# enp1s0/tsqr-gpu

Hardware: AMD Instinct MI355X
Metric: tsqr_gflops (higher is better)
Workload: dtype f32; 1 GPU; c2: M=2^20 x N=64 per GPU, fp32_tc_cor, reorth=0, U(-1,1); global 1048576 x 64 (weak scaling); F_QR=4MN^2-4/3N^3; R-factor engine: gram_bf16x3_cholesky; engine=gram_bf16x3_cholesky, m_per_gpu=1048576, n=64, mode=fp32_tc_cor, reorthogonalize=False, parallelism=row-partitioned x1

## Files before the change

### include/tsqr_mi.h

```cpp
#ifndef TSQR_MI_H
#define TSQR_MI_H
#include <stddef.h>

#ifdef __cplusplus
extern "C" {
#endif

enum tsqr_mi_compute_mode {
	TSQR_MI_FP16_NOTC = 0,
	TSQR_MI_FP16_TC_NOCOR = 1,
	TSQR_MI_FP32_NOTC = 2,
	TSQR_MI_FP32_TC_COR = 3,
	TSQR_MI_FP32_TC_NOCOR = 4,
	TSQR_MI_MIXED_TC_COR_EMU = 5,
	TSQR_MI_TF32_TC_COR = 6,
	TSQR_MI_TF32_TC_COR_EMU = 7,
	TSQR_MI_TF32_TC_NOCOR = 8,
	TSQR_MI_TF32_TC_NOCOR_EMU = 9
};

#define TSQR_MI_SUCCESS               0
#define TSQR_MI_ERROR_INVALID_SIZE    1
#define TSQR_MI_ERROR_UNSUPPORTED     2
#define TSQR_MI_ERROR_NOT_FINITE      3

int tsqr_mi_version(void);
const char* tsqr_mi_last_error(void);

size_t tsqr_mi_working_q_size(size_t m, size_t n);
size_t tsqr_mi_working_r_size(size_t m, size_t n);
size_t tsqr_mi_working_l_size(size_t m);
size_t tsqr_mi_working_reorth_size(size_t m);
size_t tsqr_mi_batch_size_log2(size_t m);
size_t tsqr_mi_batch_size(size_t m);

int tsqr_mi_qr_f32(int mode, int reorth,
                   float* q, size_t ldq, float* r, size_t ldr, float* a, size_t lda,
                   size_t m, size_t n,
                   void* wq, void* wr, float* reorth_w, unsigned* d_wl, unsigned* h_wl,
                   void* stream);
typedef struct tsqr_mi_ticket {
	int state;
	int pending;
	int slot;
	int own_flag;
	unsigned seq;
	unsigned verdict;
	float scond;
	int mode, reorth;
	float *q, *r, *a;
	size_t ldq, ldr, lda, m, n;
	void *wq, *wr, *stream;
	unsigned *h_wl, *words, *words_dev;
} tsqr_mi_ticket;
int tsqr_mi_qr_f32_submit(int mode, int reorth,
                          float* q, size_t ldq, float* r, size_t ldr, float* a, size_t lda,
                          size_t m, size_t n,
                          void* wq, void* wr, float* reorth_w, unsigned* d_wl, unsigned* h_wl,
                          void* stream, tsqr_mi_ticket* ticket);
int tsqr_mi_qr_f32_finish(tsqr_mi_ticket* ticket);

int tsqr_mi_qr_f32_loop(int count, int mode, int reorth,
                        float* q, size_t ldq, float* r, size_t ldr, float* a, size_t lda,
                        size_t m, size_t n,
                        void* wq, void* wr, float* reorth_w, unsigned* d_wl, unsigned* h_wl,
                        void* stream);
void tsqr_mi_set_loop_depth(int depth);

int tsqr_mi_qr_f32_batch(int count, int mode, int reorth,
                         float* const* q, size_t ldq, float* const* r, size_t ldr, float* const* a, size_t lda,
                         size_t m, size_t n,
                         void* wq, void* wr, float* reorth_w, unsigned* d_wl, unsigned* h_wl,
                         void* stream, int* states);

size_t tsqr_mi_working_q_size_f16(size_t m, size_t n);
size_t tsqr_mi_working_r_size_f16(size_t m, size_t n);
int tsqr_mi_qr_f16(int mode, int reorth,
                   void* q, size_t ldq, void* r, size_t ldr, const void* a, size_t lda,
                   size_t m, size_t n,
                   void* wq, void* wr, void* reorth_w, unsigned* d_wl, unsigned* h_wl,
                   void* stream);
int tsqr_mi_qr_f16_loop(int count, int mode, int reorth,
                        void* q, size_t ldq, void* r, size_t ldr, const void* a, size_t lda,
                        size_t m, size_t n,
                        void* wq, void* wr, void* reorth_w, unsigned* d_wl, unsigned* h_wl,
                        void* stream);

int tsqr_mi_qr_f16_batch(int count, int mode, int reorth,
                         void* const* q, size_t ldq, void* const* r, size_t ldr, const void* const* a, size_t lda,
                         size_t m, size_t n,
                         void* wq, void* wr, void* reorth_w, unsigned* d_wl, unsigned* h_wl,
                         void* stream, int* states);

int tsqr_mi_local_r_f32(float* r, size_t ldr, const float* a, size_t lda, size_t m, size_t n,
                        void* wq, void* wr, void* stream);
int tsqr_mi_apply_rinv_f32(int mode, float* q, size_t ldq, const float* a, size_t lda,
                           const float* r, size_t ldr, size_t m, size_t n,
                           void* wq, void* stream);
size_t tsqr_mi_gram_elems(size_t n);
int tsqr_mi_gram_f32(int level, double* gsum, const float* a, size_t lda, size_t m, size_t n, void* wq, void* wr, void* stream);
int tsqr_mi_chol_f32(int level, float* r, size_t ldr, const double* gsum, size_t m, size_t n, void* wq, unsigned* status_out, void* stream);
int tsqr_mi_chol_status(const void* wq, size_t m, size_t n, unsigned* status_out, void* stream);
int tsqr_mi_stream_wait(void* stream);
int tsqr_mi_apply_z_f32(int mode, float* q, size_t ldq, const float* a, size_t lda, size_t m, size_t n, void* wq, void* stream);
int tsqr_mi_rmul_f32(float* r, size_t ldr, const float* r2, size_t ldr2, size_t n, void* wq, void* stream);

size_t tsqr_mi_working_q_size_dist(size_t m_local, size_t n, int nranks);
size_t tsqr_mi_working_r_size_dist(size_t m_local, size_t n, int nranks);
int tsqr_mi_qr_f32_dist(int mode, int reorth,
                        float* q, size_t ldq, float* r, size_t ldr, float* a, size_t lda,
                        size_t m_local, size_t n,
                        void* wq, void* wr, float* gather_buf ,
                        void* nccl_comm, int nranks, void* stream);
int tsqr_mi_qr_f32_dist_fn(int mode, int reorth,
                           float* q, size_t ldq, float* r, size_t ldr, float* a, size_t lda,
                           size_t m_local, size_t n,
                           void* wq, void* wr, float* gather_buf ,
                           void* nccl_comm, void* nccl_allreduce_fn, void* nccl_allgather_fn, int nranks, void* stream);
int tsqr_mi_qr_f32_dist_fn_loop(int count, int mode, int reorth,
                                float* q, size_t ldq, float* r, size_t ldr, float* a, size_t lda,
                                size_t m_local, size_t n,
                                void* wq, void* wr, float* gather_buf,
                                void* nccl_comm, void* nccl_allreduce_fn, void* nccl_allgather_fn, int nranks, void* stream);
int tsqr_mi_qr_f32_dist_fn_batch(int count, int mode, int reorth,
                                 float* const* q, size_t ldq, float* const* r, size_t ldr, float* const* a, size_t lda,
                                 size_t m_local, size_t n,
                                 void* wq, void* wr, float* gather_buf,
                                 void* nccl_comm, void* nccl_allreduce_fn, void* nccl_allgather_fn, int nranks, void* stream, int* states);
typedef int (*tsqr_mi_allreduce_f64_cb)(void* user, double* buf , size_t count, void* stream);
typedef int (*tsqr_mi_allgather_f32_cb)(void* user, const float* send , float* recv , size_t count, void* stream);
int tsqr_mi_qr_f32_dist_cb(int mode, int reorth,
                           float* q, size_t ldq, float* r, size_t ldr, float* a, size_t lda,
                           size_t m_local, size_t n,
                           void* wq, void* wr, float* gather_buf,
                           tsqr_mi_allreduce_f64_cb allreduce, tsqr_mi_allgather_f32_cb allgather, void* user, int nranks, void* stream);
int tsqr_mi_qr_f32_dist_cb_loop(int count, int mode, int reorth,
                                float* q, size_t ldq, float* r, size_t ldr, float* a, size_t lda,
                                size_t m_local, size_t n,
                                void* wq, void* wr, float* gather_buf,
                                tsqr_mi_allreduce_f64_cb allreduce, tsqr_mi_allgather_f32_cb allgather, void* user, int nranks, void* stream);
int tsqr_mi_qr_f32_dist_cb_batch(int count, int mode, int reorth,
                                 float* const* q, size_t ldq, float* const* r, size_t ldr, float* const* a, size_t lda,
                                 size_t m_local, size_t n,
                                 void* wq, void* wr, float* gather_buf,
                                 tsqr_mi_allreduce_f64_cb allreduce, tsqr_mi_allgather_f32_cb allgather, void* user, int nranks, void* stream, int* states);

size_t tsqr_mi_working_q_size_f64(size_t m, size_t n);
size_t tsqr_mi_working_r_size_f64(size_t m, size_t n);
int tsqr_mi_qr_f64(int reorth, double* q, size_t ldq, double* r, size_t ldr, double* a, size_t lda,
                   size_t m, size_t n, void* wq, void* wr, void* stream);
int tsqr_mi_last_sweeps_f64(void);

size_t tsqr_mi_working_q_size_f64_wide(size_t m, size_t n);
size_t tsqr_mi_working_r_size_f64_wide(size_t m, size_t n);
int tsqr_mi_qr_f64_wide(int reorth, double* q, size_t ldq, double* r, size_t ldr, double* a, size_t lda,
                        size_t m, size_t n, void* wq, void* wr, void* stream);

int tsqr_mi_validate_f32(const float* q, size_t ldq, const float* r, size_t ldr, const float* a, size_t lda,
                         size_t m, size_t n, double* scratch, double* out_host, double* gram_out_host, void* stream);

void tsqr_mi_profile_enable(int on);
int tsqr_mi_profile_read(double* ms, long* launches, int max_classes);

void tsqr_mi_set_policy(int policy);
int tsqr_mi_last_engine(void);

void tsqr_mi_set_tuning(int level0_waves, int tree_chunks_per_wave);
void tsqr_mi_set_tuning2(int gram_waves, int apply_waves);

#ifdef __cplusplus
}
#endif
#endif
```

### tsqr_gpu_amd/blockqr.py

```python
import ctypes
import enum
import os

_HERE = os.path.dirname(os.path.abspath(__file__))
LIB_PATH = os.environ.get("TSQR_MI_LIB") or os.path.join(_HERE, "csrc", "libtsqr_mi.so")


class compute_mode(enum.IntEnum):
    fp16_notc = 0
    fp16_tc_nocor = 1
    fp32_notc = 2
    fp32_tc_cor = 3
    fp32_tc_nocor = 4
    mixed_tc_cor_emu = 5
    tf32_tc_cor = 6
    tf32_tc_cor_emu = 7
    tf32_tc_nocor = 8
    tf32_tc_nocor_emu = 9


tsqr_colmun_size = 16
success_factorization = 0
error_invalid_matrix_size = 1
error_unsupported_mode = 2
error_not_finite = 3

C_ABI_SYMBOLS = [
    "tsqr_mi_version", "tsqr_mi_last_error",
    "tsqr_mi_working_q_size", "tsqr_mi_working_r_size", "tsqr_mi_working_l_size",
    "tsqr_mi_working_reorth_size", "tsqr_mi_batch_size_log2", "tsqr_mi_batch_size",
    "tsqr_mi_qr_f32", "tsqr_mi_local_r_f32", "tsqr_mi_apply_rinv_f32", "tsqr_mi_rmul_f32",
    "tsqr_mi_qr_f32_dist", "tsqr_mi_set_tuning", "tsqr_mi_profile_enable", "tsqr_mi_profile_read",
    "tsqr_mi_set_policy", "tsqr_mi_last_engine", "tsqr_mi_set_tuning2",
    "tsqr_mi_gram_elems", "tsqr_mi_gram_f32", "tsqr_mi_chol_f32", "tsqr_mi_chol_status", "tsqr_mi_stream_wait", "tsqr_mi_apply_z_f32", "tsqr_mi_validate_f32",
    "tsqr_mi_working_q_size_dist", "tsqr_mi_working_r_size_dist", "tsqr_mi_qr_f32_dist_cb",
    "tsqr_mi_qr_f32_loop", "tsqr_mi_qr_f32_dist_fn", "tsqr_mi_qr_f32_dist_fn_loop", "tsqr_mi_qr_f32_dist_cb_loop",
    "tsqr_mi_qr_f16", "tsqr_mi_qr_f16_loop", "tsqr_mi_working_q_size_f16", "tsqr_mi_working_r_size_f16",
    "tsqr_mi_qr_f32_submit", "tsqr_mi_qr_f32_finish", "tsqr_mi_set_loop_depth", "tsqr_mi_qr_f32_batch", "tsqr_mi_qr_f16_batch",
    "tsqr_mi_qr_f32_dist_fn_batch", "tsqr_mi_qr_f32_dist_cb_batch",
    "tsqr_mi_qr_f64", "tsqr_mi_working_q_size_f64", "tsqr_mi_working_r_size_f64", "tsqr_mi_last_sweeps_f64",
    "tsqr_mi_qr_f64_wide", "tsqr_mi_working_q_size_f64_wide", "tsqr_mi_working_r_size_f64_wide",
]


class Ticket(ctypes.Structure):
    _fields_ = [("state", ctypes.c_int), ("pending", ctypes.c_int), ("slot", ctypes.c_int), ("own_flag", ctypes.c_int), ("seq", ctypes.c_uint),
                ("verdict", ctypes.c_uint), ("scond", ctypes.c_float), ("mode", ctypes.c_int), ("reorth", ctypes.c_int),
                ("q", ctypes.c_void_p), ("r", ctypes.c_void_p), ("a", ctypes.c_void_p),
                ("ldq", ctypes.c_size_t), ("ldr", ctypes.c_size_t), ("lda", ctypes.c_size_t), ("m", ctypes.c_size_t), ("n", ctypes.c_size_t),
                ("wq", ctypes.c_void_p), ("wr", ctypes.c_void_p), ("stream", ctypes.c_void_p),
                ("h_wl", ctypes.c_void_p), ("words", ctypes.c_void_p), ("words_dev", ctypes.c_void_p)]

    def __del__(self):
        if self.pending == 0:
            return
        import sys
        import threading
        if _lib is not None and not sys.is_finalizing() and getattr(self, "_tid", None) == threading.get_ident():
            _lib.tsqr_mi_qr_f32_finish(ctypes.byref(self))
        else:
            import warnings
            warnings.warn("tsqr_gpu_amd: a Ticket in flight was dropped on another thread (or at shutdown) without finish(); "
                          "call blockqr.finish(ticket) on the submitting thread", ResourceWarning, stacklevel=2)


FP16_MODES = (compute_mode.fp16_notc, compute_mode.fp16_tc_nocor)

_lib = None


def lib():
    global _lib
    if _lib is not None:
        return _lib
    if not os.path.exists(LIB_PATH):
        raise RuntimeError(
            "tsqr_gpu_amd: %s is missing -- build it with `python -c 'import __graft_entry__ as g; g.build()'` "
            "or `make -C tsqr_gpu_amd/csrc`. There is no CPU fallback." % LIB_PATH)
    import torch
    L = ctypes.CDLL(LIB_PATH)
    sz, vp, ci = ctypes.c_size_t, ctypes.c_void_p, ctypes.c_int
    L.tsqr_mi_version.restype = ci
    L.tsqr_mi_last_error.restype = ctypes.c_char_p
    for name, args in [("tsqr_mi_working_q_size", [sz, sz]), ("tsqr_mi_working_r_size", [sz, sz]),
                       ("tsqr_mi_working_l_size", [sz]), ("tsqr_mi_working_reorth_size", [sz]),
                       ("tsqr_mi_batch_size_log2", [sz]), ("tsqr_mi_batch_size", [sz])]:
        getattr(L, name).restype = sz
        getattr(L, name).argtypes = args
    L.tsqr_mi_qr_f32.restype = ci
    L.tsqr_mi_qr_f32.argtypes = [ci, ci, vp, sz, vp, sz, vp, sz, sz, sz, vp, vp, vp, vp, vp, vp]
    L.tsqr_mi_local_r_f32.restype = ci
    L.tsqr_mi_local_r_f32.argtypes = [vp, sz, vp, sz, sz, sz, vp, vp, vp]
    L.tsqr_mi_apply_rinv_f32.restype = ci
    L.tsqr_mi_apply_rinv_f32.argtypes = [ci, vp, sz, vp, sz, vp, sz, sz, sz, vp, vp]
    L.tsqr_mi_gram_elems.restype = sz
    L.tsqr_mi_gram_elems.argtypes = [sz]
    L.tsqr_mi_gram_f32.restype = ci
    L.tsqr_mi_gram_f32.argtypes = [ci, vp, vp, sz, sz, sz, vp, vp, vp]
    L.tsqr_mi_chol_f32.restype = ci
    L.tsqr_mi_chol_f32.argtypes = [ci, vp, sz, vp, sz, sz, vp, ctypes.POINTER(ctypes.c_uint), vp]
    L.tsqr_mi_chol_status.restype = ci
    L.tsqr_mi_chol_status.argtypes = [vp, sz, sz, ctypes.POINTER(ctypes.c_uint), vp]
    L.tsqr_mi_stream_wait.restype = ci
    L.tsqr_mi_stream_wait.argtypes = [vp]
    L.tsqr_mi_apply_z_f32.restype = ci
    L.tsqr_mi_apply_z_f32.argtypes = [ci, vp, sz, vp, sz, sz, sz, vp, vp]
    L.tsqr_mi_validate_f32.restype = ci
    L.tsqr_mi_validate_f32.argtypes = [vp, sz, vp, sz, vp, sz, sz, sz, vp, ctypes.POINTER(ctypes.c_double), ctypes.POINTER(ctypes.c_double), vp]
    L.tsqr_mi_rmul_f32.restype = ci
    L.tsqr_mi_rmul_f32.argtypes = [vp, sz, vp, sz, sz, vp, vp]
    L.tsqr_mi_qr_f32_dist.restype = ci
    L.tsqr_mi_qr_f32_dist.argtypes = [ci, ci, vp, sz, vp, sz, vp, sz, sz, sz, vp, vp, vp, vp, ci, vp]
    L.tsqr_mi_qr_f32_dist_cb.restype = ci
    L.tsqr_mi_qr_f32_dist_cb.argtypes = [ci, ci, vp, sz, vp, sz, vp, sz, sz, sz, vp, vp, vp, vp, vp, vp, ci, vp]
    L.tsqr_mi_qr_f32_loop.restype = ci
    L.tsqr_mi_qr_f32_loop.argtypes = [ci] + L.tsqr_mi_qr_f32.argtypes
    L.tsqr_mi_qr_f32_submit.restype = ci
    L.tsqr_mi_qr_f32_submit.argtypes = L.tsqr_mi_qr_f32.argtypes + [ctypes.POINTER(Ticket)]
    L.tsqr_mi_qr_f32_finish.restype = ci
    L.tsqr_mi_qr_f32_finish.argtypes = [ctypes.POINTER(Ticket)]
    L.tsqr_mi_qr_f32_batch.restype = ci
    L.tsqr_mi_qr_f32_batch.argtypes = [ci, ci, ci, vp, sz, vp, sz, vp, sz, sz, sz, vp, vp, vp, vp, vp, vp, vp]
    L.tsqr_mi_qr_f16_batch.restype = ci
    L.tsqr_mi_qr_f16_batch.argtypes = L.tsqr_mi_qr_f32_batch.argtypes
    L.tsqr_mi_set_loop_depth.restype = None
    L.tsqr_mi_set_loop_depth.argtypes = [ci]
    L.tsqr_mi_qr_f16.restype = ci
    L.tsqr_mi_qr_f16.argtypes = L.tsqr_mi_qr_f32.argtypes
    L.tsqr_mi_qr_f16_loop.restype = ci
    L.tsqr_mi_qr_f16_loop.argtypes = [ci] + L.tsqr_mi_qr_f32.argtypes
    for name in ("tsqr_mi_working_q_size_f16", "tsqr_mi_working_r_size_f16"):
        getattr(L, name).restype = sz
        getattr(L, name).argtypes = [sz, sz]
    L.tsqr_mi_qr_f32_dist_fn.restype = ci
    L.tsqr_mi_qr_f32_dist_fn.argtypes = [ci, ci, vp, sz, vp, sz, vp, sz, sz, sz, vp, vp, vp, vp, vp, vp, ci, vp]
    L.tsqr_mi_qr_f32_dist_fn_loop.restype = ci
    L.tsqr_mi_qr_f32_dist_fn_loop.argtypes = [ci] + L.tsqr_mi_qr_f32_dist_fn.argtypes
    L.tsqr_mi_qr_f32_dist_cb_loop.restype = ci
    L.tsqr_mi_qr_f32_dist_cb_loop.argtypes = [ci] + L.tsqr_mi_qr_f32_dist_cb.argtypes
    L.tsqr_mi_qr_f32_dist_fn_batch.restype = ci
    L.tsqr_mi_qr_f32_dist_fn_batch.argtypes = [ci, ci, ci, vp, sz, vp, sz, vp, sz, sz, sz, vp, vp, vp, vp, vp, vp, ci, vp, vp]
    L.tsqr_mi_qr_f32_dist_cb_batch.restype = ci
    L.tsqr_mi_qr_f32_dist_cb_batch.argtypes = [ci, ci, ci, vp, sz, vp, sz, vp, sz, sz, sz, vp, vp, vp, vp, vp, vp, ci, vp, vp]
    for name in ("tsqr_mi_working_q_size_dist", "tsqr_mi_working_r_size_dist"):
        getattr(L, name).restype = sz
        getattr(L, name).argtypes = [sz, sz, ci]
    L.tsqr_mi_profile_enable.restype = None
    L.tsqr_mi_profile_enable.argtypes = [ci]
    L.tsqr_mi_profile_read.restype = ci
    L.tsqr_mi_profile_read.argtypes = [ctypes.POINTER(ctypes.c_double), ctypes.POINTER(ctypes.c_long), ci]
    L.tsqr_mi_set_policy.restype = None
    L.tsqr_mi_set_policy.argtypes = [ci]
    L.tsqr_mi_last_engine.restype = ci
    L.tsqr_mi_set_tuning2.restype = None
    L.tsqr_mi_set_tuning2.argtypes = [ci, ci]
    L.tsqr_mi_set_tuning.restype = None
    L.tsqr_mi_set_tuning.argtypes = [ci, ci]
    for name in ("tsqr_mi_working_q_size_f64", "tsqr_mi_working_r_size_f64", "tsqr_mi_working_q_size_f64_wide", "tsqr_mi_working_r_size_f64_wide"):
        getattr(L, name).restype = sz
        getattr(L, name).argtypes = [sz, sz]
    for name in ("tsqr_mi_qr_f64", "tsqr_mi_qr_f64_wide"):
        getattr(L, name).restype = ci
        getattr(L, name).argtypes = [ci, vp, sz, vp, sz, vp, sz, sz, sz, vp, vp, vp]
    L.tsqr_mi_last_sweeps_f64.restype = ci
    L.tsqr_mi_last_sweeps_f64.argtypes = []
    _lib = L
    return L


def last_error():
    return lib().tsqr_mi_last_error().decode()


def get_working_q_size(m, n):
    return lib().tsqr_mi_working_q_size(m, n)


def get_working_r_size(m, n):
    return lib().tsqr_mi_working_r_size(m, n)


def get_working_l_size(m):
    return lib().tsqr_mi_working_l_size(m)
# ... 336 lines not shown
```

### tsqr_gpu_amd/csrc/tsqr_kernels.hip

```cpp
#include <hip/hip_runtime.h>
#include <stdint.h>
#include <type_traits>
#include <utility>

namespace tsqrmi {

typedef float f32x4 __attribute__((ext_vector_type(4)));
typedef float f32x4u __attribute__((ext_vector_type(4), aligned(4)));
typedef short bf16x8 __attribute__((ext_vector_type(8)));
typedef _Float16 f16x8 __attribute__((ext_vector_type(8)));
typedef _Float16 f16x4 __attribute__((ext_vector_type(4)));

__device__ __forceinline__ void lds_barrier() { asm volatile("s_waitcnt lgkmcnt(0)\n\ts_barrier" ::: "memory"); }

template <int I, int N, class F>
__device__ __forceinline__ void static_for(F&& f) {
	if constexpr (I < N) {
		f(std::integral_constant<int, I>{});
		static_for<I + 1, N>(f);
	}
}

template <int K>
__device__ __forceinline__ float bcast16(float x) {
// ... 425 lines not shown

	float p[NT][16];
	const int ch_end = min(a.nchunks, (gw + 1) * a.cpw);
	int ch_first = gw * a.cpw;
	if (TRI && ch_first < ch_end) {
		load_chunk<NT>(p, a.src, a.ld, (size_t)ch_first * 64, a.m, a.n, c, q);
#pragma unroll
		for (int ct = 0; ct < NT; ct++)
#pragma unroll
			for (int rho = 0; rho < 16; rho++) {
				const int row = 16 * (rho >> 2) + 4 * q + (rho & 3), col = 16 * ct + c;
				if (col >= row) Rw[row * NP - (row * (row - 1)) / 2 + col - row] = p[ct][rho];
			}
		ch_first++;
		__builtin_amdgcn_wave_barrier();
	}
	for (int ch = ch_first; ch < ch_end; ch++) {
		load_chunk<NT>(p, a.src, a.ld, (size_t)ch * 64, a.m, a.n, c, q);
		fold_one<NT, TRI, COR>(p, Rw, Tl, a.n, c, q);
	}
	store_packed_r<NP>(a.dst + (size_t)gw * a.rows_store, a.dst_ld, Rw, a.rows_store, a.cols_store, lane);
}

struct FoldTreeArgs {
	const float* src; size_t ld;
	int nblocks, n;
	float* dst; size_t dst_ld;
	int rows_store, cols_store;
};
constexpr int FOLD_COOP_LDS_FLOATS = FOLD_COOP_WAVES * ((64 * 65) / 2 + 16) + FOLD_COOP_WAVES * 256 + 2 * FOLD_COOP_WAVES * 64 + 3 * FOLD_COOP_WAVES * 256;
template <bool COR>
__global__ __launch_bounds__(64 * FOLD_COOP_WAVES) void fold_coop_kernel(const FoldTreeArgs a) {
	constexpr int NT = 4, NP = 64, WAVES = FOLD_COOP_WAVES;
	constexpr int RP = (NP * (NP + 1)) / 2 + 16;
	extern __shared__ __attribute__((aligned(16))) char coop_smem[];
	float* Rs = reinterpret_cast<float*>(coop_smem);
	float* Ts = Rs + WAVES * RP;
	CoopCtx cc;
	cc.xd = Ts + WAVES * 256;
	cc.xw = cc.xd + 2 * WAVES * 64;
	const int lane = threadIdx.x & 63;
	const int wv = __builtin_amdgcn_readfirstlane(threadIdx.x >> 6);
	cc.wave = wv; cc.step = 0;
	const int c = lane & 15, q = lane >> 4;
	float* Rw = Rs + wv * RP;
	float* Tl = Ts + wv * 256;
	for (int i = lane; i < RP; i += 64) Rw[i] = 0.0f;
	const int first = blockIdx.x * WAVES;
	const size_t mrows = (size_t)a.nblocks * 64;
	float p[NT][16];
	load_chunk<NT, true>(p, a.src, a.ld, (size_t)first * 64, mrows, a.n, c, q);
#pragma unroll
	for (int ct = 0; ct < NT; ct++)
#pragma unroll
		for (int rho = 0; rho < 16; rho++) {
			const int row = 16 * (rho >> 2) + 4 * q + (rho & 3), col = 16 * ct + c;
			if (col >= row) Rw[row * NP - (row * (row - 1)) / 2 + col - row] = p[ct][rho];
		}
	if (wv > 0 && first + wv < a.nblocks) {
		load_chunk<NT, true>(p, a.src, a.ld, (size_t)(first + wv) * 64, mrows, a.n, c, q);
	} else {
#pragma unroll
		for (int ct = 0; ct < NT; ct++)
#pragma unroll
			for (int rho = 0; rho < 16; rho++) p[ct][rho] = 0.0f;
	}
	__builtin_amdgcn_wave_barrier();
	fold_one<NT, true, COR, true>(p, Rw, Tl, a.n, c, q, &cc);
	if (wv == 0) store_packed_r<NP>(a.dst + (size_t)blockIdx.x * a.rows_store, a.dst_ld, Rw, a.rows_store, a.cols_store, lane);
}

typedef double f64x4 __attribute__((ext_vector_type(4)));

__device__ __forceinline__ void part_store(double* p, double v) { __builtin_nontemporal_store(v, p); }
__device__ __forceinline__ double part_load(const double* p) { return __builtin_nontemporal_load(p); }

struct GramArgs {
	const float* a; size_t lda; size_t m; int n;
	int nchunks; int cpw; int nwaves;
	double* part;
	const unsigned* skip_status;
	unsigned* announce; unsigned announce_seq;
	int old_share;
};

__device__ __forceinline__ void announce_previous_call(unsigned* word, unsigned seq) {
	if (word && blockIdx.x == 0 && threadIdx.x == 0) *reinterpret_cast<volatile unsigned*>(word) = seq;
}

template <int NT>
__global__ __launch_bounds__(256) void gram_kernel(const GramArgs a) {
	constexpr int NTRI = (NT * (NT + 1)) / 2;
	__shared__ double red[2][NTRI * 256];
	announce_previous_call(a.announce, a.announce_seq);
	if (a.skip_status && a.skip_status[0] != 0) return;
	const int lane = threadIdx.x & 63;
	const int wv = threadIdx.x >> 6;
	const int gw = blockIdx.x * 4 + wv;
	const int c = lane & 15, q = lane >> 4;
	f64x4 acc[NTRI];
#pragma unroll
	for (int t = 0; t < NTRI; t++) acc[t] = f64x4{0.0, 0.0, 0.0, 0.0};
	if (gw < a.nwaves) {
		float p[NT][16];
		const int ch_end = a.nchunks, ch_step = a.nwaves, ch_begin = gw;
		for (int ch = ch_begin; ch < ch_end; ch += ch_step) {
			load_chunk<NT>(p, a.a, a.lda, (size_t)ch * 64, a.m, a.n, c, q);
#pragma unroll
			for (int rho = 0; rho < 16; rho++) {
				double pd[NT];
#pragma unroll
				for (int t = 0; t < NT; t++) pd[t] = (double)p[t][rho];
				int idx = 0;
#pragma unroll
				for (int ti = 0; ti < NT; ti++)
#pragma unroll
					for (int tj = ti; tj < NT; tj++) {
						acc[idx] = __builtin_amdgcn_mfma_f64_16x16x4f64(pd[ti], pd[tj], acc[idx], 0, 0, 0);
						idx++;
					}
			}
		}
	}
	if (wv >= 2) {
#pragma unroll
		for (int t = 0; t < NTRI; t++)
#pragma unroll
			for (int r = 0; r < 4; r++) red[wv - 2][(t * 4 + r) * 64 + lane] = acc[t][r];
	}
	__syncthreads();
	if (wv < 2) {
#pragma unroll
		for (int t = 0; t < NTRI; t++)
#pragma unroll
			for (int r = 0; r < 4; r++) acc[t][r] += red[wv][(t * 4 + r) * 64 + lane];
	}
	__syncthreads();
	if (wv == 1) {
#pragma unroll
		for (int t = 0; t < NTRI; t++)
#pragma unroll
			for (int r = 0; r < 4; r++) red[0][(t * 4 + r) * 64 + lane] = acc[t][r];
	}
	__syncthreads();
	if (wv == 0) {
		double* out = a.part + (size_t)blockIdx.x * NTRI * 256;
#pragma unroll
		for (int t = 0; t < NTRI; t++)
#pragma unroll
			for (int r = 0; r < 4; r++) part_store(&out[(t * 4 + r) * 64 + lane], acc[t][r] + red[0][(t * 4 + r) * 64 + lane]);
	}
}

template <int NT>
__global__ __launch_bounds__(256) void gram_bf16_kernel(const GramArgs a) {
	constexpr int NTRI = (NT * (NT + 1)) / 2;
	__shared__ double red[2][NTRI * 256];
	announce_previous_call(a.announce, a.announce_seq);
	if (a.skip_status && a.skip_status[0] != 0) return;
	const int lane = threadIdx.x & 63;
	const int wv = threadIdx.x >> 6;
	const int gw = blockIdx.x * 4 + wv;
	const int c = lane & 15, q = lane >> 4;
	f32x4 acc[NTRI];
	f64x4 tot[NTRI];
#pragma unroll
	for (int t = 0; t < NTRI; t++) {
		acc[t] = f32x4{0.f, 0.f, 0.f, 0.f};
		tot[t] = f64x4{0.0, 0.0, 0.0, 0.0};
	}
	if (gw < a.nwaves) {
		float p[NT][16];
		const int ch_end = a.nchunks, ch_step = a.nwaves, ch_begin = gw;
		for (int ch = ch_begin; ch < ch_end; ch += ch_step) {
			load_chunk<NT>(p, a.a, a.lda, (size_t)ch * 64, a.m, a.n, c, q);
#pragma unroll
			for (int kt = 0; kt < 2; kt++) {
				bf16x8 oh[NT], om[NT], ol[NT];
#pragma unroll
				for (int t = 0; t < NT; t++) {
					u32x4 hh, mm, ll;
#pragma unroll
					for (int jp = 0; jp < 4; jp++) {
						unsigned h, m, lo;
						split3_pair(p[t][8 * kt + 2 * jp], p[t][8 * kt + 2 * jp + 1], h, m, lo);
						hh[jp] = h; mm[jp] = m; ll[jp] = lo;
					}
					oh[t] = __builtin_bit_cast(bf16x8, hh);
					om[t] = __builtin_bit_cast(bf16x8, mm);
					ol[t] = __builtin_bit_cast(bf16x8, ll);
				}
#pragma unroll
				for (int pass = 3; pass < 9; pass++) {
					int idx = 0;
#pragma unroll
					for (int ti = 0; ti < NT; ti++)
#pragma unroll
						for (int tj = ti; tj < NT; tj++) {
							const bf16x8 av = (pass == 4 || pass == 6 || pass == 8) ? oh[ti] : ((pass == 3 || pass == 7) ? om[ti] : ol[ti]);
							const bf16x8 bv = (pass == 5 || pass == 7 || pass == 8) ? oh[tj] : ((pass == 3 || pass == 6) ? om[tj] : ol[tj]);
							acc[idx] = __builtin_amdgcn_mfma_f32_16x16x32_bf16(av, bv, acc[idx], 0, 0, 0);
							idx++;
						}
				}
#pragma unroll
				for (int t = 0; t < NTRI; t++) {
#pragma unroll
					for (int r = 0; r < 4; r++) tot[t][r] += (double)acc[t][r];
					acc[t] = f32x4{0.f, 0.f, 0.f, 0.f};
				}
			}
		}
	}
	double dacc[NTRI][4];
#pragma unroll
	for (int t = 0; t < NTRI; t++)
#pragma unroll
		for (int r = 0; r < 4; r++) dacc[t][r] = (double)tot[t][r];
	if (wv >= 2) {
#pragma unroll
		for (int t = 0; t < NTRI; t++)
#pragma unroll
			for (int r = 0; r < 4; r++) red[wv - 2][(t * 4 + r) * 64 + lane] = dacc[t][r];
	}
	__syncthreads();
	if (wv < 2) {
#pragma unroll
		for (int t = 0; t < NTRI; t++)
#pragma unroll
			for (int r = 0; r < 4; r++) dacc[t][r] += red[wv][(t * 4 + r) * 64 + lane];
	}
	__syncthreads();
	if (wv == 1) {
#pragma unroll
		for (int t = 0; t < NTRI; t++)
#pragma unroll
			for (int r = 0; r < 4; r++) red[0][(t * 4 + r) * 64 + lane] = dacc[t][r];
	}
	__syncthreads();
	if (wv == 0) {
		double* out = a.part + (size_t)blockIdx.x * NTRI * 256;
// ... 21 lines not shown
#pragma unroll
		for (int t = 0; t < NT; t++)
#pragma unroll
			for (int kt = 0; kt < 2; kt++) {
				const size_t row = (size_t)ch * 64 + 32 * kt + 8 * q;
				const int col = 16 * t + c;
				f16x8 v = {0, 0, 0, 0, 0, 0, 0, 0};
				if (col < a.n) {
					const _Float16* src = A + (size_t)col * a.lda + row;
					if (row + 7 < a.m) v = *reinterpret_cast<const f16x8*>(src);
					else {
#pragma unroll
						for (int i = 0; i < 8; i++)
							if (row + i < a.m) v[i] = src[i];
					}
				}
				op[t][kt] = v;
			}
	};
	if (gw < a.nwaves) {
		f16x8 cur[NT][2], nxt[NT][2];
		int ch = gw;
		if (ch < a.nchunks) load_chunk_h(cur, ch);
		for (; ch < a.nchunks; ch += a.nwaves) {
			const bool more = ch + a.nwaves < a.nchunks;
			if (more) load_chunk_h(nxt, ch + a.nwaves);
#pragma unroll
			for (int kt = 0; kt < 2; kt++) {
				int idx = 0;
#pragma unroll
				for (int ti = 0; ti < NT; ti++)
#pragma unroll
					for (int tj = ti; tj < NT; tj++) {
						acc[idx] = __builtin_amdgcn_mfma_f32_16x16x32_f16(cur[ti][kt], cur[tj][kt], acc[idx], 0, 0, 0);
						idx++;
					}
			}
#pragma unroll
			for (int t = 0; t < NTRI; t++) {
#pragma unroll
				for (int r = 0; r < 4; r++) tot[t][r] += (double)acc[t][r];
				acc[t] = f32x4{0.f, 0.f, 0.f, 0.f};
			}
			if (more) {
#pragma unroll
				for (int t = 0; t < NT; t++) { cur[t][0] = nxt[t][0]; cur[t][1] = nxt[t][1]; }
			}
		}
	}
	if (wv >= 2) {
#pragma unroll
		for (int t = 0; t < NTRI; t++)
#pragma unroll
			for (int r = 0; r < 4; r++) red[wv - 2][(t * 4 + r) * 64 + lane] = tot[t][r];
	}
	__syncthreads();
	if (wv < 2) {
#pragma unroll
		for (int t = 0; t < NTRI; t++)
#pragma unroll
			for (int r = 0; r < 4; r++) tot[t][r] += red[wv][(t * 4 + r) * 64 + lane];
	}
	__syncthreads();
	if (wv == 1) {
#pragma unroll
		for (int t = 0; t < NTRI; t++)
#pragma unroll
			for (int r = 0; r < 4; r++) red[0][(t * 4 + r) * 64 + lane] = tot[t][r];
	}
	__syncthreads();
	if (wv == 0) {
		double* out = a.part + (size_t)wg * NTRI * 256;
#pragma unroll
		for (int t = 0; t < NTRI; t++)
#pragma unroll
			for (int r = 0; r < 4; r++) part_store(&out[(t * 4 + r) * 64 + lane], tot[t][r] + red[0][(t * 4 + r) * 64 + lane]);
	}
}
template <int NT>
__global__ __launch_bounds__(256) void gram_h_kernel(const GramArgs a) {
	constexpr int NTRI = (NT * (NT + 1)) / 2;
	__shared__ double red[2][NTRI * 256];
	announce_previous_call(a.announce, a.announce_seq);
	gram_h_body<NT>(a, red, blockIdx.x);
}

constexpr int GB_ROWS = 128, GB_RS = 136;
constexpr int GB_OLD_SHARE = 20;
constexpr int GB_LDS_BYTES = 2 * 64 * GB_RS * 4;
__device__ __forceinline__ void gram_blk_body(const GramArgs& a, float* gb_as, const int wg, const int nwg) {
	constexpr int NTRI = 10;
	static_assert(GB_LDS_BYTES >= (int)sizeof(double) * 2 * NTRI * 256, "the final workgroup reduction aliases the block buffers");
	if (a.skip_status && a.skip_status[0] != 0) return;
	const int lane = threadIdx.x & 63;
	const int wv = __builtin_amdgcn_readfirstlane(threadIdx.x >> 6);
	const int c = lane & 15, q = lane >> 4;
	const int lcol = lane >> 5, lrow = 4 * (lane & 31);
	const int nblk = a.nchunks;
	int first = wg, step = nwg, bend = nblk;
	if ((nwg & 1) == 0 && nblk >= 2 * nwg) {
		const int half = nwg >> 1, p = wg < half ? wg : wg - half;
		const int K = (nblk - p + half - 1) / half;
		const int H = (K * (a.old_share ? a.old_share : GB_OLD_SHARE) + 16) >> 5;
		step = half;
		first = wg < half ? p : p + half * H;
		bend = wg < half ? p + half * H : p + half * K;
	}
	const int blast = first < bend ? first + ((bend - 1 - first) / step) * step : min(first, nblk - 1);
	f64x4 tot[NTRI];
#pragma unroll
	for (int t = 0; t < NTRI; t++) tot[t] = f64x4{0.0, 0.0, 0.0, 0.0};
	const unsigned voff = (unsigned)(((size_t)lcol * a.lda + lrow) * sizeof(float));
	const unsigned soff0 = (unsigned)((size_t)(2 * wv) * a.lda * sizeof(float)), soffk = (unsigned)(8 * a.lda * sizeof(float));
	auto load_block = [&](f32x4 (&v)[8], int b) {
		const auto rs = __builtin_amdgcn_make_buffer_rsrc(const_cast<float*>(a.a + (size_t)min(b, blast) * GB_ROWS), 0, -1, 0x00020000);
#pragma unroll
		for (int k = 0; k < 8; k++) v[k] = __builtin_bit_cast(f32x4, __builtin_amdgcn_raw_buffer_load_b128(rs, voff, soff0 + k * soffk, 0));
	};
	auto stage = [&](const f32x4 (&v)[8], float* buf) {
#pragma unroll
		for (int k = 0; k < 8; k++) *reinterpret_cast<f32x4*>(&buf[(2 * wv + lcol + 8 * k) * GB_RS + lrow]) = v[k];
	};
	auto products = [&](const float* buf) {
		bf16x8 oh[4], om[4], ol[4];
#pragma unroll
		for (int t = 0; t < 4; t++) {
			const float* src = &buf[(16 * t + c) * GB_RS + 32 * wv + 8 * q];
			const f32x4 x0 = *reinterpret_cast<const f32x4*>(src), x1 = *reinterpret_cast<const f32x4*>(src + 4);
			u32x4 hh, mm, ll;
			unsigned h, m, lo;
			split3_pair(x0[0], x0[1], h, m, lo); hh[0] = h; mm[0] = m; ll[0] = lo;
			split3_pair(x0[2], x0[3], h, m, lo); hh[1] = h; mm[1] = m; ll[1] = lo;
			split3_pair(x1[0], x1[1], h, m, lo); hh[2] = h; mm[2] = m; ll[2] = lo;
			split3_pair(x1[2], x1[3], h, m, lo); hh[3] = h; mm[3] = m; ll[3] = lo;
			oh[t] = __builtin_bit_cast(bf16x8, hh);
			om[t] = __builtin_bit_cast(bf16x8, mm);
			ol[t] = __builtin_bit_cast(bf16x8, ll);
		}
		static_for<0, 2>([&](auto gg) {
			constexpr int g = decltype(gg)::value;
			f32x4 acc[5];
#pragma unroll
			for (int i = 0; i < 5; i++) acc[i] = f32x4{0.f, 0.f, 0.f, 0.f};
#pragma unroll
			for (int pass = 3; pass < 9; pass++)
				static_for<0, 5>([&](auto ii) {
					constexpr int idx = 5 * g + decltype(ii)::value;
					constexpr int ti = idx < 4 ? 0 : (idx < 7 ? 1 : (idx < 9 ? 2 : 3));
					constexpr int tj = idx < 4 ? idx : (idx < 7 ? idx - 3 : (idx < 9 ? idx - 5 : 3));
					const bf16x8 av = (pass == 4 || pass == 6 || pass == 8) ? oh[ti] : ((pass == 3 || pass == 7) ? om[ti] : ol[ti]);
					const bf16x8 bv = (pass == 5 || pass == 7 || pass == 8) ? oh[tj] : ((pass == 3 || pass == 6) ? om[tj] : ol[tj]);
					acc[idx - 5 * g] = __builtin_amdgcn_mfma_f32_16x16x32_bf16(av, bv, acc[idx - 5 * g], 0, 0, 0);
				});
#pragma unroll
			for (int i = 0; i < 5; i++)
#pragma unroll
				for (int r = 0; r < 4; r++) tot[5 * g + i][r] += (double)acc[i][r];
		});
	};
	constexpr int BUF = 64 * GB_RS;
	f32x4 vx[8], vy[8];
	int bi = first, it = 0;
	load_block(vx, bi);
	asm volatile("" ::: "memory");
	load_block(vy, bi + step);
	asm volatile("" ::: "memory");
	if (bi < bend) stage(vx, gb_as);
	while (bi < bend) {
		lds_barrier();
		load_block(vx, bi + 2 * step);
		asm volatile("" ::: "memory");
		products(gb_as + (it & 1) * BUF);
		bi += step; it++;
		if (bi >= bend) break;
		stage(vy, gb_as + (it & 1) * BUF);
		lds_barrier();
		load_block(vy, bi + 2 * step);
		asm volatile("" ::: "memory");
		products(gb_as + (it & 1) * BUF);
		bi += step; it++;
		if (bi >= bend) break;
		stage(vx, gb_as + (it & 1) * BUF);
	}
	__syncthreads();
	double* red = reinterpret_cast<double*>(gb_as);
	if (wv >= 2) {
#pragma unroll
		for (int t = 0; t < NTRI; t++)
#pragma unroll
			for (int r = 0; r < 4; r++) red[(wv - 2) * NTRI * 256 + (t * 4 + r) * 64 + lane] = tot[t][r];
	}
	__syncthreads();
	if (wv < 2) {
#pragma unroll
		for (int t = 0; t < NTRI; t++)
#pragma unroll
			for (int r = 0; r < 4; r++) tot[t][r] += red[wv * NTRI * 256 + (t * 4 + r) * 64 + lane];
	}
	__syncthreads();
	if (wv == 1) {
#pragma unroll
		for (int t = 0; t < NTRI; t++)
#pragma unroll
			for (int r = 0; r < 4; r++) red[(t * 4 + r) * 64 + lane] = tot[t][r];
	}
	__syncthreads();
	if (wv == 0) {
		double* out = a.part + (size_t)wg * NTRI * 256;
#pragma unroll
		for (int t = 0; t < NTRI; t++)
#pragma unroll
			for (int r = 0; r < 4; r++) part_store(&out[(t * 4 + r) * 64 + lane], tot[t][r] + red[(t * 4 + r) * 64 + lane]);
	}
}
__global__ __launch_bounds__(256, 2) void gram_blk_kernel(const GramArgs a) {
	extern __shared__ __attribute__((aligned(16))) float gb_as[];
	announce_previous_call(a.announce, a.announce_seq);
	gram_blk_body(a, gb_as, blockIdx.x, gridDim.x);
}

template <bool WT = false>
__device__ __forceinline__ void gram_reduce1_body(const int blk, double (*red)[17], double* __restrict__ gout, const double* __restrict__ part,
                                                  int nparts, int nelem, double rows, float* __restrict__ fin_r, size_t fin_ldr,
                                                  float* __restrict__ fin_zneg, int fin_ny) {
	if (blk == 0 && threadIdx.x == 0) gout[nelem] = rows;
	const int e = threadIdx.x & 15, s = threadIdx.x >> 4;
	const int el = blk * 16 + e;
	double s0 = 0.0, s1 = 0.0, s2 = 0.0, s3 = 0.0;
	if (el < nelem) {
		auto head = [&](auto uu) {
			constexpr int U = decltype(uu)::value;
			double v[U];
#pragma unroll
			for (int u = 0; u < U; u++) {
				const int b = s + 16 * u;
				v[u] = part_load(&part[(size_t)min(b, nparts - 1) * nelem + el]);
			}
#pragma unroll
			for (int u = 0; u < U; u++)
				if (s + 16 * u >= nparts) v[u] = 0.0;
#pragma unroll
			for (int u = 0; u < U; u++) {
				if ((u & 3) == 0) s0 += v[u];
				else if ((u & 3) == 1) s1 += v[u];
				else if ((u & 3) == 2) s2 += v[u];
				else s3 += v[u];
			}
		};
		if (nparts <= 16) head(std::integral_constant<int, 1>{});
		else if (nparts <= 32) head(std::integral_constant<int, 2>{});
		else if (nparts <= 64) head(std::integral_constant<int, 4>{});
		else if (nparts <= 128) head(std::integral_constant<int, 8>{});
		else if (nparts <= 256) head(std::integral_constant<int, 16>{});
		else head(std::integral_constant<int, 32>{});
		for (int b = s + 512; b < nparts; b += 16) s0 += part_load(&part[(size_t)b * nelem + el]);
	}
	red[s][e] = (s0 + s1) + (s2 + s3);
	__syncthreads();
	if (s == 0 && el < nelem) {
		double v[16];
#pragma unroll
		for (int k = 0; k < 16; k++) v[k] = red[k][e];
		const double sum = ((v[0] + v[1]) + (v[2] + v[3])) + ((v[4] + v[5]) + (v[6] + v[7])) +
		                   (((v[8] + v[9]) + (v[10] + v[11])) + ((v[12] + v[13]) + (v[14] + v[15])));
		if (WT) __hip_atomic_store(&gout[el], sum, __ATOMIC_RELAXED, __HIP_MEMORY_SCOPE_AGENT);
		else gout[el] = sum;
		if (fin_zneg) {
			const int t = el >> 8, reg = (el >> 6) & 3, l = el & 63;
			const int i = 16 * (t >> 2) + 4 * (l >> 4) + reg, j = 16 * (t & 3) + (l & 15);
			const float f = (float)sum;
			fin_zneg[(size_t)j * 64 + i] = (j < fin_ny) ? -f : 0.0f;
			if (j < fin_ny) fin_r[(size_t)j * fin_ldr + i] = f;
		}
	}
}
__global__ __launch_bounds__(256) void gram_reduce1_kernel(double* __restrict__ gout, const double* __restrict__ part, int nparts, int nelem,
                                                           double rows, float* __restrict__ fin_r = nullptr, size_t fin_ldr = 0,
                                                           float* __restrict__ fin_zneg = nullptr, int fin_ny = 0) {
	__shared__ double red[16][17];
	gram_reduce1_body<false>(blockIdx.x, red, gout, part, nparts, nelem, rows, fin_r, fin_ldr, fin_zneg, fin_ny);
}

__device__ __forceinline__ double bcast_lane_f64(double x, int lane_const) {
	const unsigned long long u = __builtin_bit_cast(unsigned long long, x);
	const unsigned lo = __builtin_amdgcn_readlane((unsigned)u, lane_const);
	const unsigned hi = __builtin_amdgcn_readlane((unsigned)(u >> 32), lane_const);
	return __builtin_bit_cast(double, ((unsigned long long)hi << 32) | lo);
}

#ifdef TSQR_CHOL_STAMPS
__device__ unsigned long long* g_chol_stamp_out = nullptr;
constexpr int CHOL_NSTAMP = 160;
__shared__ unsigned long long chol_stamp_lds[4 * CHOL_NSTAMP];
#define CHOL_STAMP16(slot) do { if ((threadIdx.x & 63) == 0 && (threadIdx.x >> 6) < 4) chol_stamp_lds[(threadIdx.x >> 6) * CHOL_NSTAMP + (slot)] = __builtin_amdgcn_s_memtime(); } while (0)
#else
#define CHOL_STAMP16(slot) do {} while (0)
#endif
typedef double f64x2c __attribute__((ext_vector_type(2)));

__device__ __forceinline__ void chol_section4(double (&g)[4], double (&mm)[4], const int K0, const int j, const int n,
                                              double (&rk)[4], double (&mk)[4], double (&piv0)[4], double* __restrict__ rr, double* __restrict__ mr) {
	double a00 = bcast_lane_f64(g[0], K0);
	double a10 = bcast_lane_f64(g[1], K0), a11 = bcast_lane_f64(g[1], K0 + 1);
	double a20 = bcast_lane_f64(g[2], K0), a21 = bcast_lane_f64(g[2], K0 + 1), a22 = bcast_lane_f64(g[2], K0 + 2);
	double a30 = bcast_lane_f64(g[3], K0), a31 = bcast_lane_f64(g[3], K0 + 1), a32 = bcast_lane_f64(g[3], K0 + 2), a33 = bcast_lane_f64(g[3], K0 + 3);
	auto inv_sqrt = [](double piv) {
		double y = __builtin_amdgcn_rsq(piv);
		return fma(0.5 * y, fma(-piv * y, y, 1.0), y);
	};
	const bool live0 = K0 < n, live1 = K0 + 1 < n, live2 = K0 + 2 < n, live3 = K0 + 3 < n;
	piv0[0] = a00;
	const double p0 = (a00 > 0.0) ? a00 : 1.0;
	const double y0 = inv_sqrt(p0);
	const double l10 = live0 ? a10 * y0 : 0.0, l20 = live0 ? a20 * y0 : 0.0, l30 = live0 ? a30 * y0 : 0.0;
	rk[0] = !live0 ? 0.0 : ((j > K0) ? g[0] * y0 : ((j == K0) ? p0 * y0 : 0.0));
	mk[0] = live0 ? mm[0] * y0 : 0.0;
	rr[0 * 64 + j] = rk[0]; mr[0 * 64 + j] = mk[0];
	a11 = fma(-l10, l10, a11); a21 = fma(-l20, l10, a21); a31 = fma(-l30, l10, a31);
	a22 = fma(-l20, l20, a22); a32 = fma(-l30, l20, a32); a33 = fma(-l30, l30, a33);
	g[1] = fma(-l10, rk[0], g[1]); mm[1] = fma(-l10, mk[0], mm[1]);
	g[2] = fma(-l20, rk[0], g[2]); mm[2] = fma(-l20, mk[0], mm[2]);
	g[3] = fma(-l30, rk[0], g[3]); mm[3] = fma(-l30, mk[0], mm[3]);
	piv0[1] = a11;
	const double p1 = (a11 > 0.0) ? a11 : 1.0;
	const double y1 = inv_sqrt(p1);
	const double l21 = live1 ? a21 * y1 : 0.0, l31 = live1 ? a31 * y1 : 0.0;
	rk[1] = !live1 ? 0.0 : ((j > K0 + 1) ? g[1] * y1 : ((j == K0 + 1) ? p1 * y1 : 0.0));
	mk[1] = live1 ? mm[1] * y1 : 0.0;
	rr[1 * 64 + j] = rk[1]; mr[1 * 64 + j] = mk[1];
	a22 = fma(-l21, l21, a22); a32 = fma(-l31, l21, a32); a33 = fma(-l31, l31, a33);
	g[2] = fma(-l21, rk[1], g[2]); mm[2] = fma(-l21, mk[1], mm[2]);
	g[3] = fma(-l31, rk[1], g[3]); mm[3] = fma(-l31, mk[1], mm[3]);
	piv0[2] = a22;
	const double p2 = (a22 > 0.0) ? a22 : 1.0;
	const double y2 = inv_sqrt(p2);
	const double l32 = live2 ? a32 * y2 : 0.0;
	rk[2] = !live2 ? 0.0 : ((j > K0 + 2) ? g[2] * y2 : ((j == K0 + 2) ? p2 * y2 : 0.0));
	mk[2] = live2 ? mm[2] * y2 : 0.0;
	rr[2 * 64 + j] = rk[2]; mr[2 * 64 + j] = mk[2];
	a33 = fma(-l32, l32, a33);
	g[3] = fma(-l32, rk[2], g[3]); mm[3] = fma(-l32, mk[2], mm[3]);
	piv0[3] = a33;
	const double p3 = (a33 > 0.0) ? a33 : 1.0;
	const double y3 = inv_sqrt(p3);
	rk[3] = !live3 ? 0.0 : ((j > K0 + 3) ? g[3] * y3 : ((j == K0 + 3) ? p3 * y3 : 0.0));
	mk[3] = live3 ? mm[3] * y3 : 0.0;
	rr[3 * 64 + j] = rk[3]; mr[3 * 64 + j] = mk[3];
}

template <class OT, class LOADG>
__device__ __forceinline__ void chol_body16(OT* __restrict__ r, size_t ldr, OT* __restrict__ z, unsigned* __restrict__ status,
                                            unsigned* __restrict__ host_status, LOADG loadg, int n, int NT, int f32_layout, float min_ratio,
                                            float max_scond, double shift_coef = 0.0, double min_diag = 0.0, double** gs_out = nullptr) {
	__shared__ double Gs[64 * 65];
	if (gs_out) *gs_out = Gs;
	__shared__ double Rrow[2 * 256], Mrow[2 * 256], dg[64], pv[64], sred[16];
	const int t = threadIdx.x;
	const int j = t & 63, w = __builtin_amdgcn_readfirstlane(t >> 6);
	const int NP = 16 * NT;
	CHOL_STAMP16(0);
#ifdef TSQR_CHOL_STAMPS
	if ((threadIdx.x & 63) == 0 && w < 4) chol_stamp_lds[w * CHOL_NSTAMP + 5] = __builtin_amdgcn_s_memrealtime();
#endif
// ... 88 lines not shown
#pragma unroll 1
	for (int gi = 0; gi < ngroups; gi++) {
		CHOL_STAMP16(8 + 8 * gi + 1);
		lds_barrier();
		CHOL_STAMP16(8 + 8 * gi + 2);
		if (w == gi + 1 && gi + 1 < ngroups) {
			update(gi);
			CHOL_STAMP16(8 + 8 * gi + 4);
			section(gi + 1);
			CHOL_STAMP16(8 + 8 * gi + 7);
		} else if (w > gi) {
			update(gi);
		}
		if (w == ((gi + 15) & 15)) {
			const int K0 = 4 * gi;
			const double* rr = Rrow + (gi & 1) * 256;
			const double* mr = Mrow + (gi & 1) * 256;
#pragma unroll
			for (int u = 0; u < 4; u++) {
				const int K = K0 + u;
				const double rkj = rr[u * 64 + j], mkc = mr[u * 64 + j];
				if (K < n) {
					if (j < NP) z[(size_t)K * NP + j] = (j <= K) ? (OT)mkc : (OT)0;
					if (j < n) r[(size_t)j * ldr + K] = (j >= K) ? (OT)rkj : (OT)0;
					Gs[K * 65 + j] = (j <= K) ? mkc : 0.0;
					if (j <= K) s_acc = fma(dgj * mkc, mkc, s_acc);
				}
			}
		}
		CHOL_STAMP16(8 + 8 * gi + 3);
	}
	CHOL_STAMP16(2);
	for (int o = 32; o > 0; o >>= 1) s_acc += __shfl_xor(s_acc, o);
	if (j == 0) sred[w] = s_acc;
	lds_barrier();
	if (w == 0) {
		const double d0 = dg[j], p0 = pv[j];
		float ratio = (j < n) ? ((d0 > 0.0) ? (float)(p0 / d0) : 0.0f) : 1.0f;
		if (j < n && !(d0 >= min_diag)) ratio = 0.0f;
		for (int o = 32; o > 0; o >>= 1) ratio = fminf(ratio, __shfl_xor(ratio, o));
		if (j == 0) {
			double ssum = 0.0;
#pragma unroll
			for (int k = 0; k < 16; k++) ssum += sred[k];
			const float scond = (float)(ssum / (double)n);
			const unsigned s0 = (ratio > min_ratio && scond <= max_scond) ? 0u : 1u;
			status[0] = s0;
			status[1] = __builtin_bit_cast(unsigned, ratio);
			status[2] = __builtin_bit_cast(unsigned, scond);
			if (host_status) {
				volatile unsigned* hs = host_status;
				hs[1] = __builtin_bit_cast(unsigned, ratio);
				hs[2] = __builtin_bit_cast(unsigned, scond);
				hs[0] = s0;
			}
		}
	}
	CHOL_STAMP16(3);
#ifdef TSQR_CHOL_STAMPS
	if ((threadIdx.x & 63) == 0 && w < 4) chol_stamp_lds[w * CHOL_NSTAMP + 4] = __builtin_amdgcn_s_memrealtime();
	__syncthreads();
	if (g_chol_stamp_out)
		for (int i = threadIdx.x; i < 4 * CHOL_NSTAMP; i += 1024) g_chol_stamp_out[i] = chol_stamp_lds[i];
#endif
}

struct CholArgs {
	float* r; size_t ldr;
	float* z;
	unsigned* status;
	unsigned* host_status;
	const double* gsum;
	const unsigned* prev_status;
	const double* rows_dev;
	double rows;
	double shift_coef;
	int n, NT;
	int level;
	float scond_floor;
	int relax;
	int retry_shift;
};

__global__ __launch_bounds__(1024) void chol16_kernel(const CholArgs a) {
	if (a.prev_status && a.prev_status[0] != 0) {
		if (threadIdx.x == 0) {
			a.status[0] = 1u; a.status[1] = 0u; a.status[2] = 0u;
			if (a.host_status) { volatile unsigned* hs = a.host_status; hs[1] = 0u; hs[2] = 0u; hs[0] = 1u; }
		}
		return;
	}
	const double rows = a.rows_dev ? a.rows_dev[0] : a.rows;
	float min_ratio = 0.0f, max_scond = INFINITY;
	double min_diag = 0.0, shift = 0.0;
	if (a.level == 2) {
		min_ratio = 0.03125f;
		max_scond = fminf(128.0f, fmaxf(a.scond_floor, 0.12f * sqrtf((float)rows)));
		min_diag = rows * 0x1p-90;
		if (a.relax) { min_ratio = 0x1p-20f; max_scond = fminf(1.6e7f, 8000.0f * sqrtf((float)rows)); }
	} else if (a.level == 1) {
		min_ratio = 9.094947017729282e-13f;
	} else {
		shift = a.shift_coef * (rows * (double)a.n + (double)a.n * (double)(a.n + 1));
	}
	const bool retry = a.level == 2 && a.retry_shift != 0;
	auto loadg = [&](int e) { return a.gsum[e]; };
	chol_body16(a.r, a.ldr, a.z, a.status, retry ? nullptr : a.host_status, loadg, a.n, a.NT, a.level == 2 ? 1 : 0, min_ratio, max_scond, shift, min_diag);
	if (!retry) return;
	__shared__ unsigned again;
	__syncthreads();
	if (threadIdx.x == 0) { again = a.status[0]; a.status[3] = 0u; }
	__syncthreads();
	if (again) {
		const double coef = 8.0 * 0x1p-23 / sqrt(fmax(rows, 1.0));
		chol_body16(a.r, a.ldr, a.z, a.status, nullptr, loadg, a.n, a.NT, 1, 0.0f, INFINITY, coef, min_diag);
		__syncthreads();
		if (threadIdx.x == 0 && a.status[0] == 0u) a.status[3] = 1u;
	}
	if (threadIdx.x == 0 && a.host_status) {
		volatile unsigned* hs = a.host_status;
		hs[1] = a.status[1];
		hs[2] = a.status[2];
		hs[0] = (a.status[0] == 0u && a.status[3] != 0u) ? 2u : a.status[0];
	}
}

template <int U>
__device__ __forceinline__ void chol_group4(double (&g)[16], double (&mm)[16], double* Rrow, double* Mrow, float* __restrict__ r, size_t ldr,
                                           float* __restrict__ z, int NP, double* Zd,
                                           double* pv, int w, int j, int n, int kk, double dgj, double& s_acc) {
	const int K0 = 16 * kk + 4 * U;
	if (K0 >= n) return;
	double* rr = Rrow + (U & 1) * 256;
	double* mr = Mrow + (U & 1) * 256;
	if (w == U) {
		double g4[4] = {g[0], g[1], g[2], g[3]}, m4[4] = {mm[0], mm[1], mm[2], mm[3]};
		double rk[4], mk[4], piv0[4];
		chol_section4(g4, m4, K0, j, n, rk, mk, piv0, rr, mr);
#pragma unroll
		for (int u = 0; u < 4; u++) {
			g[u] = g4[u]; mm[u] = m4[u];
			if (j == 0 && K0 + u < n) pv[K0 + u] = piv0[u];
		}
	}
	lds_barrier();
	double rkj[4], mkc[4];
#pragma unroll
	for (int u = 0; u < 4; u++) { rkj[u] = rr[u * 64 + j]; mkc[u] = mr[u * 64 + j]; }
	if (w == ((U + 3) & 3)) {
#pragma unroll
		for (int u = 0; u < 4; u++) {
			const int K = K0 + u;
			if (K < n) {
				if (j < NP) z[(size_t)K * NP + j] = (j <= K) ? (float)mkc[u] : 0.0f;
				if (j < n) r[(size_t)j * ldr + K] = (j >= K) ? (float)rkj[u] : 0.0f;
				Zd[K * 65 + j] = (j <= K) ? mkc[u] : 0.0;
				if (j <= K) s_acc = fma(dgj * mkc[u], mkc[u], s_acc);
			}
		}
	}
	const int nlive = 16 - 4 * kk;
#pragma unroll
	for (int s = 0; s < 16; s++) {
		if (s < nlive && !(s < 4 && w <= U)) {
			const int i = 16 * (kk + (s >> 2)) + 4 * w + (s & 3);
			double acc_g = g[s], acc_m = mm[s];
#pragma unroll
			for (int u = 0; u < 4; u++) {
				const double rki = rr[u * 64 + i];
				acc_g = fma(-rki, rkj[u], acc_g);
				acc_m = fma(-rki, mkc[u], acc_m);
			}
			g[s] = acc_g; mm[s] = acc_m;
		}
	}
}

template <class LOADG>
__device__ __forceinline__ void chol_body4(float* __restrict__ r, size_t ldr, float* __restrict__ z, unsigned* __restrict__ status,
                                          unsigned* __restrict__ host_status, LOADG loadg, int n, int NT, int f32_layout, float min_ratio,
                                          float max_scond, double shift_coef, double min_diag, double* lds) {
	double* Gs = lds;
	double* Rrow = Gs + 64 * 65;
	double* Mrow = Rrow + 2 * 256;
	double* dg = Mrow + 2 * 256;
	double* pv = dg + 64;
	const int t = threadIdx.x;
	const int j = t & 63, w = t >> 6;
	const int NP = 16 * NT;
	double gv[10];
	{
		int idx = 0;
		for (int ti = 0; ti < 4; ti++)
			for (int tj = ti; tj < 4; tj++) {
				if (ti < NT && tj < NT) { gv[ti * 4 + tj - (ti * (ti + 1)) / 2] = loadg(idx * 256 + t); idx++; }
				else gv[ti * 4 + tj - (ti * (ti + 1)) / 2] = 0.0;
			}
	}
	if (NT < 4)
		for (int i = t; i < 64 * 65; i += 256) Gs[i] = 0.0;
	for (int e = n * NP + t; e < NP * NP; e += 256) z[e] = 0.0f;
	__syncthreads();
	{
		const int reg = t >> 6, l = t & 63;
#pragma unroll
		for (int ti = 0; ti < 4; ti++)
#pragma unroll
			for (int tj = ti; tj < 4; tj++) {
				if (ti < NT && tj < NT) {
					const int row = 16 * ti + (f32_layout ? 4 * (l >> 4) + reg : (l >> 4) + 4 * reg);
					const int col = 16 * tj + (l & 15);
					const double v = gv[ti * 4 + tj - (ti * (ti + 1)) / 2];
					if (row <= col) {
						Gs[row * 65 + col] = v;
						Gs[col * 65 + row] = v;
					}
				}
			}
	}
	__syncthreads();
	if (shift_coef > 0.0) {
		if (w == 0) {
			double tr = (j < n) ? Gs[j * 65 + j] : 0.0;
			for (int o = 32; o > 0; o >>= 1) tr += __shfl_xor(tr, o);
			if (j < n) Gs[j * 65 + j] += shift_coef * tr;
		}
		__syncthreads();
	}
	double g[16], mm[16];
#pragma unroll
	for (int s = 0; s < 16; s++) {
		const int i = 16 * (s >> 2) + 4 * w + (s & 3);
		g[s] = Gs[i * 65 + j];
		mm[s] = (i == j) ? 1.0 : 0.0;
	}
	if (t < 64) { dg[t] = Gs[t * 65 + t]; pv[t] = 1.0; }
	const double dgj = Gs[j * 65 + j];
	double s_acc = 0.0;
	__syncthreads();
#pragma unroll 1
	for (int kk = 0; kk < 4; kk++) {
		static_for<0, 4>([&](auto u) { chol_group4<decltype(u)::value>(g, mm, Rrow, Mrow, r, ldr, z, NP, Gs, pv, w, j, n, kk, dgj, s_acc); });
#pragma unroll
		for (int s = 0; s < 12; s++) { g[s] = g[s + 4]; mm[s] = mm[s + 4]; }
	}
	for (int o = 32; o > 0; o >>= 1) s_acc += __shfl_xor(s_acc, o);
	__syncthreads();
	if (j == 0) Rrow[w] = s_acc;
	__syncthreads();
	if (w == 0) {
		const double d0 = dg[j], p0 = pv[j];
		float ratio = (j < n) ? ((d0 > 0.0) ? (float)(p0 / d0) : 0.0f) : 1.0f;
		if (j < n && !(d0 >= min_diag)) ratio = 0.0f;
		for (int o = 32; o > 0; o >>= 1) ratio = fminf(ratio, __shfl_xor(ratio, o));
		if (j == 0) {
			const float scond = (float)(((Rrow[0] + Rrow[1]) + (Rrow[2] + Rrow[3])) / (double)n);
			const unsigned s0 = (ratio > min_ratio && scond <= max_scond) ? 0u : 1u;
			status[0] = s0;
			status[1] = __builtin_bit_cast(unsigned, ratio);
			status[2] = __builtin_bit_cast(unsigned, scond);
			if (host_status) {
				volatile unsigned* hs = host_status;
				hs[1] = __builtin_bit_cast(unsigned, ratio);
				hs[2] = __builtin_bit_cast(unsigned, scond);
				hs[0] = s0;
			}
		}
	}
}


#if defined(__HIP_DEVICE_COMPILE__) && !defined(__gfx950__) && !defined(__gfx942__)
#error "tsqr_kernels.hip: the chained launches rely on gfx942 / gfx950 memory-counter semantics (vmcnt covers stores); port the hand-over before building for another target"
#endif
struct ChainArgs {
	CholArgs chol;
	const double* part; int nparts;
	unsigned* ticket;
	int nred;
	int direct;
};
__global__ __launch_bounds__(256, 2) void gram_blk_chain_kernel(const GramArgs a, const ChainArgs ch) {
	extern __shared__ __attribute__((aligned(16))) float gb_as[];
	static_assert(GB_LDS_BYTES >= (int)sizeof(double) * (64 * 65 + 4 * 256 + 128), "chol_body4's arrays alias the block buffers");
	announce_previous_call(a.announce, a.announce_seq);
	const int nchain = ch.direct ? 1 : ch.nred;
	if ((int)blockIdx.x >= nchain) {
		gram_blk_body(a, gb_as, (int)blockIdx.x - nchain, (int)gridDim.x - nchain);
		return;
	}
	const CholArgs& c = ch.chol;
	if (ch.direct) {
		const double rows = c.rows_dev ? c.rows_dev[0] : c.rows;
		const float max_scond = fminf(128.0f, fmaxf(c.scond_floor, 0.12f * sqrtf((float)rows)));
		const double* g = c.gsum;
		chol_body4(c.r, c.ldr, c.z, c.status, c.host_status, [&](int e) { return g[e]; }, c.n, c.NT, 1, 0.03125f, max_scond, 0.0,
		           rows * 0x1p-90, reinterpret_cast<double*>(gb_as));
		return;
	}
	gram_reduce1_body<true>(blockIdx.x, reinterpret_cast<double (*)[17]>(gb_as), const_cast<double*>(c.gsum), ch.part, ch.nparts, 10 * 256, c.rows,
	                        nullptr, 0, nullptr, 0);
	asm volatile("s_waitcnt vmcnt(0)" ::: "memory");
	__syncthreads();
	__shared__ unsigned last;
	if (threadIdx.x == 0) last = (__hip_atomic_fetch_add(ch.ticket, 1u, __ATOMIC_RELAXED, __HIP_MEMORY_SCOPE_AGENT) == (unsigned)(ch.nred - 1)) ? 1u : 0u;
	__syncthreads();
	if (!last) return;
	if (threadIdx.x == 0) __hip_atomic_store(ch.ticket, 0u, __ATOMIC_RELAXED, __HIP_MEMORY_SCOPE_AGENT);
	const double rows = c.rows;
	const float max_scond = fminf(128.0f, fmaxf(c.scond_floor, 0.12f * sqrtf((float)rows)));
	const double* g = c.gsum;
	chol_body4(c.r, c.ldr, c.z, c.status, c.host_status, [&](int e) { return __hip_atomic_load(&g[e], __ATOMIC_RELAXED, __HIP_MEMORY_SCOPE_AGENT); }, c.n, c.NT, 1, 0.03125f, max_scond, 0.0,
	           rows * 0x1p-90, reinterpret_cast<double*>(gb_as));
}

__global__ __launch_bounds__(256) void gram_h_chain_kernel(const GramArgs a, const ChainArgs ch) {
	__shared__ double hc_lds[64 * 65 + 4 * 256 + 128];
	static_assert(sizeof(hc_lds) >= sizeof(double) * 2 * 10 * 256, "the Gram role's workgroup sum fits");
	announce_previous_call(a.announce, a.announce_seq);
	if ((int)blockIdx.x >= ch.nred) {
		gram_h_body<4>(a, reinterpret_cast<double (*)[10 * 256]>(hc_lds), (int)blockIdx.x - ch.nred);
		return;
	}
	const CholArgs& c = ch.chol;
	gram_reduce1_body<true>(blockIdx.x, reinterpret_cast<double (*)[17]>(hc_lds), const_cast<double*>(c.gsum), ch.part, ch.nparts, 10 * 256, c.rows,
	                        nullptr, 0, nullptr, 0);
	asm volatile("s_waitcnt vmcnt(0)" ::: "memory");
	__syncthreads();
	__shared__ unsigned last;
	if (threadIdx.x == 0) last = (__hip_atomic_fetch_add(ch.ticket, 1u, __ATOMIC_RELAXED, __HIP_MEMORY_SCOPE_AGENT) == (unsigned)(ch.nred - 1)) ? 1u : 0u;
	__syncthreads();
	if (!last) return;
	if (threadIdx.x == 0) __hip_atomic_store(ch.ticket, 0u, __ATOMIC_RELAXED, __HIP_MEMORY_SCOPE_AGENT);
	const double rows = c.rows;
	const float max_scond = fminf(128.0f, fmaxf(c.scond_floor, 0.12f * sqrtf((float)rows)));
	const double* g = c.gsum;
	chol_body4(c.r, c.ldr, c.z, c.status, c.host_status, [&](int e) { return __hip_atomic_load(&g[e], __ATOMIC_RELAXED, __HIP_MEMORY_SCOPE_AGENT); }, c.n, c.NT,
	           1, 0.03125f, max_scond, 0.0, rows * 0x1p-90, hc_lds);
}

struct CrossArgs {
	const float* x; size_t ldx; const float* y; size_t ldy; size_t m; int ny;
	int nchunks; int cpw; int nwaves;
	double* part;
	int ny_total;
};

__global__ __launch_bounds__(256, 2) void cross_kernel(const CrossArgs a) {
	__shared__ float red[2][16 * 256];
	const int lane = threadIdx.x & 63;
	const int wv = threadIdx.x >> 6;
	const int gw = blockIdx.x * 4 + wv;
	const int c = lane & 15, q = lane >> 4;
	const float* const ypan = a.y + (size_t)blockIdx.y * 64 * a.ldy;
	const int ny = a.ny_total > 0 ? min(64, a.ny_total - 64 * (int)blockIdx.y) : a.ny;
	f32x4 acc[16];
#pragma unroll
	for (int t = 0; t < 16; t++) acc[t] = f32x4{0.f, 0.f, 0.f, 0.f};
	if (gw < a.nwaves) {
		const int ch_end = min(a.nchunks, (gw + 1) * a.cpw);
		for (int ch = gw * a.cpw; ch < ch_end; ch++) {
			float px[4][16], py[4][16];
			load_chunk<4>(px, a.x, a.ldx, (size_t)ch * 64, a.m, 64, c, q);
			load_chunk<4>(py, ypan, a.ldy, (size_t)ch * 64, a.m, ny, c, q);
#pragma unroll
			for (int kt = 0; kt < 2; kt++) {
				bf16x8 xh[4], xm[4], xl[4], yh[4], ym[4], yl[4];
#pragma unroll
				for (int t = 0; t < 4; t++) {
					u32x4 hh, mm, ll;
#pragma unroll
					for (int jp = 0; jp < 4; jp++) {
						unsigned h, m, lo;
						split3_pair(px[t][8 * kt + 2 * jp], px[t][8 * kt + 2 * jp + 1], h, m, lo);
						hh[jp] = h; mm[jp] = m; ll[jp] = lo;
					}
					xh[t] = __builtin_bit_cast(bf16x8, hh); xm[t] = __builtin_bit_cast(bf16x8, mm); xl[t] = __builtin_bit_cast(bf16x8, ll);
#pragma unroll
					for (int jp = 0; jp < 4; jp++) {
						unsigned h, m, lo;
						split3_pair(py[t][8 * kt + 2 * jp], py[t][8 * kt + 2 * jp + 1], h, m, lo);
						hh[jp] = h; mm[jp] = m; ll[jp] = lo;
					}
					yh[t] = __builtin_bit_cast(bf16x8, hh); ym[t] = __builtin_bit_cast(bf16x8, mm); yl[t] = __builtin_bit_cast(bf16x8, ll);
				}
#pragma unroll
				for (int pass = 3; pass < 9; pass++)
#pragma unroll
					for (int ti = 0; ti < 4; ti++)
#pragma unroll
						for (int tj = 0; tj < 4; tj++) {
							const bf16x8 av = (pass == 4 || pass == 6 || pass == 8) ? xh[ti] : ((pass == 3 || pass == 7) ? xm[ti] : xl[ti]);
							const bf16x8 bv = (pass == 5 || pass == 7 || pass == 8) ? yh[tj] : ((pass == 3 || pass == 6) ? ym[tj] : yl[tj]);
							acc[4 * ti + tj] = __builtin_amdgcn_mfma_f32_16x16x32_bf16(av, bv, acc[4 * ti + tj], 0, 0, 0);
						}
			}
		}
	}
	if (wv >= 2) {
#pragma unroll
		for (int t = 0; t < 16; t++)
#pragma unroll
			for (int r = 0; r < 4; r++) red[wv - 2][(t * 4 + r) * 64 + lane] = acc[t][r];
	}
	__syncthreads();
	if (wv < 2) {
#pragma unroll
		for (int t = 0; t < 16; t++)
#pragma unroll
			for (int r = 0; r < 4; r++) acc[t][r] += red[wv][(t * 4 + r) * 64 + lane];
	}
	__syncthreads();
	if (wv == 1) {
#pragma unroll
		for (int t = 0; t < 16; t++)
#pragma unroll
			for (int r = 0; r < 4; r++) red[0][(t * 4 + r) * 64 + lane] = acc[t][r];
	}
	__syncthreads();
	if (wv == 0) {
		double* out = a.part + ((size_t)blockIdx.y * gridDim.x + blockIdx.x) * 16 * 256;
#pragma unroll
		for (int t = 0; t < 16; t++)
#pragma unroll
			for (int r = 0; r < 4; r++) part_store(&out[(t * 4 + r) * 64 + lane], (double)(acc[t][r] + red[0][(t * 4 + r) * 64 + lane]));
	}
}

constexpr int CROSS_GSTRIDE = 16 * 256 + 8;
__global__ __launch_bounds__(256) void cross_reduce_multi_kernel(double* __restrict__ gout, const double* __restrict__ part, int nparts, double rows,
                                                                 float* __restrict__ fin_r, size_t fin_ldr, float* __restrict__ fin_zneg, int ny_total) {
	__shared__ double red[16][17];
	const int j = blockIdx.y;
	gram_reduce1_body<false>(blockIdx.x, red, gout + (size_t)j * CROSS_GSTRIDE, part + (size_t)j * nparts * (16 * 256), nparts, 16 * 256, rows,
	                         fin_zneg ? fin_r + (size_t)j * 64 * fin_ldr : nullptr, fin_ldr, fin_zneg ? fin_zneg + (size_t)j * 4096 : nullptr,
	                         min(64, ny_total - 64 * j));
}

__global__ __launch_bounds__(256) void cross_finish_kernel(float* __restrict__ r, size_t ldr, float* __restrict__ zneg,
                                                           const double* __restrict__ gsum, int ny, int ny_total = 0) {
	if (ny_total > 0) {
		const int j = blockIdx.y;
		r += (size_t)j * 64 * ldr; zneg += (size_t)j * 4096; gsum += (size_t)j * CROSS_GSTRIDE; ny = min(64, ny_total - 64 * j);
	}
	for (int e = blockIdx.x * 256 + threadIdx.x; e < 16 * 256; e += 256 * gridDim.x) {
		const int t = e >> 8, reg = (e >> 6) & 3, l = e & 63;
		const int i = 16 * (t >> 2) + 4 * (l >> 4) + reg;
		const int j = 16 * (t & 3) + (l & 15);
		const float v = (float)gsum[e];
		zneg[(size_t)j * 64 + i] = (j < ny) ? -v : 0.0f;
		if (j < ny) r[(size_t)j * ldr + i] = v;
	}
}

template <int U>
__device__ __forceinline__ void trinv_group(double (&mm)[16], double* Mrow, const double* Rs, const double* rdiag,
                                            float* __restrict__ z, int w, int j, int n, int NP, int kk) {
	const int K0 = 16 * kk + 4 * U;
	if (K0 >= n) return;
	double* mr = Mrow + (U & 1) * 256;
	if (w == U) {
		static_for<0, 4>([&](auto uu) {
			constexpr int u = decltype(uu)::value;
			const int K = K0 + u;
			const bool live = K < n;
			const double mk = live ? mm[u] * rdiag[K] : 0.0;
			static_for<u + 1, 4>([&](auto vv) {
				constexpr int v = decltype(vv)::value;
				mm[v] = fma(-Rs[K * 65 + K0 + v], mk, mm[v]);
			});
			mr[u * 64 + j] = mk;
			if (live && j < NP) z[(size_t)K * NP + j] = (j <= K) ? (float)mk : 0.0f;
		});
	}
	__syncthreads();
	double mkc[4];
#pragma unroll
	for (int u = 0; u < 4; u++) mkc[u] = mr[u * 64 + j];
	const int nlive = 16 - 4 * kk;
#pragma unroll
	for (int s = 0; s < 16; s++) {
		if (s < nlive && !(s < 4 && w <= U)) {
			const int i = 16 * (kk + (s >> 2)) + 4 * w + (s & 3);
			double acc = mm[s];
#pragma unroll
			for (int u = 0; u < 4; u++) acc = fma(-Rs[(K0 + u) * 65 + i], mkc[u], acc);
			mm[s] = acc;
		}
	}
}

__global__ __launch_bounds__(256) void trinv_kernel(float* __restrict__ z, const float* __restrict__ r, size_t ldr,
                                                    int n, int NP) {
	__shared__ double Rs[64 * 65];
	__shared__ double Mrow[2 * 256], rdiag[64];
	const int t = threadIdx.x;
	const int j = t & 63, w = t >> 6;
	for (int e = t; e < 64 * 64; e += 256) {
		const int row = e & 63, col = e >> 6;
		Rs[row * 65 + col] = (row <= col && col < n) ? (double)r[(size_t)col * ldr + row] : 0.0;
	}
	for (int e = n * NP + t; e < NP * NP; e += 256) z[e] = 0.0f;
	__syncthreads();
	if (t < 64) rdiag[t] = (t < n) ? 1.0 / Rs[t * 65 + t] : 0.0;
	double mm[16];
#pragma unroll
	for (int s = 0; s < 16; s++) mm[s] = (16 * (s >> 2) + 4 * w + (s & 3) == j) ? 1.0 : 0.0;
	__syncthreads();
#pragma unroll 1
	for (int kk = 0; kk < 4; kk++) {
		static_for<0, 4>([&](auto u) { trinv_group<decltype(u)::value>(mm, Mrow, Rs, rdiag, z, w, j, n, NP, kk); });
#pragma unroll
		for (int s = 0; s < 12; s++) mm[s] = mm[s + 4];
	}
}

struct ApplyArgs {
	const float* a; size_t lda; float* q; size_t ldq; size_t m; int n;
	const float* z;
	int nchunks; int cpw; int nwaves;
	int n_out;
	int multi_cols;
	double* gpart;
	const unsigned* skip_status;
	const float* r32; void* r16; size_t ldr16;
	int share[4];
	int even_share;
	int plain_q;
	int forward;
};

template <int ENGINE, int NT, bool UPD, int ROWS, bool GRAMQ, int NW = 4, class IO = float>
__device__ __forceinline__ void apply_wg_body(const ApplyArgs& a) {
	static_assert(!GRAMQ || NW == 4, "the fused Gram accumulation is written for four waves");
	static_assert(sizeof(IO) == 4 || (!UPD && !GRAMQ), "fp16 I/O: the plain product only");
	constexpr int NP = 16 * NT;
	constexpr int RS = ROWS + 4;
	constexpr int LPC = ROWS / 4, CPI = 64 / LPC;
	constexpr int NI = NP / (NW * CPI);
	constexpr int SL = ROWS / (16 * NW);
	constexpr int ZS = NP + 16;
	constexpr bool ZTRI = (ENGINE == 0 && NT == 8 && !UPD);
	auto ztri_stride = [](int g) { return g == 0 ? 144 : (g <= 2 ? 112 : (g <= 4 ? 80 : (g <= 6 ? 48 : 16))); };
	auto ztri_base = [&](int g) { int o = 0; for (int i = 0; i < g; i++) o += 16 * ztri_stride(i); return o; };
	constexpr int KT = (NP + 31) / 32;
	constexpr bool COMPACT = (!UPD && (NT == 4 || NT == 8));
	constexpr int NB = COMPACT ? KT * NT - KT * (KT - 1) : KT * NT;
	auto zblk = [](int kt, int ct) { return COMPACT ? kt * NT - kt * (kt - 1) + ct - 2 * kt : kt * NT + ct; };
	auto zblk_kt = [](int b) { int kt = 0; while (COMPACT && kt + 1 < KT && b >= (kt + 1) * NT - (kt + 1) * kt) kt++; return COMPACT ? kt : b / NT; };
	extern __shared__ __attribute__((aligned(16))) char smem[];
	float* As = reinterpret_cast<float*>(smem);
	char* zbase = smem + sizeof(float) * NP * RS;
	const int lane = threadIdx.x & 63;
	const int wv = threadIdx.x >> 6;
	const int c = lane & 15, q = lane >> 4;
	const int lcol = lane / LPC, lrow = 4 * (lane % LPC);

	const int nblk = a.nchunks, nwg = a.nwaves;
	auto swz = [](int col) { return ((col >> 3) & 1) << 4; };
	auto load_block = [&](f32x4 (&v)[NI], const auto* base, size_t ld, int ncols, int b) {
		using T = std::remove_cv_t<std::remove_pointer_t<decltype(base)>>;
		const size_t row = (size_t)b * ROWS + lrow;
#pragma unroll
		for (int k = 0; k < NI; k++) {
			const int col = (wv + NW * k) * CPI + lcol;
			v[k] = f32x4{0.f, 0.f, 0.f, 0.f};
			if (col < ncols) {
				const T* src = base + (size_t)col * ld + row;
				if (row + 3 < a.m) {
					if constexpr (sizeof(T) == 2) {
						const f16x4 h = *reinterpret_cast<const f16x4*>(src);
						v[k] = f32x4{(float)h[0], (float)h[1], (float)h[2], (float)h[3]};
					} else {
						v[k] = *reinterpret_cast<const f32x4u*>(src);
					}
				} else {
#pragma unroll
					for (int i = 0; i < 4; i++)
						if (row + i < a.m) v[k][i] = (float)src[i];
				}
			}
		}
	};
	const IO* a_in = reinterpret_cast<const IO*>(a.a);

	constexpr int NTRI = (NT * (NT + 1)) / 2;
	f64x4 gtot[GRAMQ ? NTRI : 1];
	if constexpr (GRAMQ) {
#pragma unroll
		for (int t = 0; t < NTRI; t++) gtot[t] = f64x4{0.0, 0.0, 0.0, 0.0};
	}
	constexpr bool DEEP = (ROWS == 64 && !UPD) || NW == 8 || sizeof(IO) == 2;
	f32x4 v[NI], v2[DEEP ? NI : 1];
	const int quarter = nwg >> 2;
	constexpr bool CAN_SHARE = !UPD && !GRAMQ && ROWS == 64 && NW == 4 && sizeof(IO) == 4;
	const bool uneven = CAN_SHARE && a.share[0] != 0 && (nwg & 7) == 0 && nblk % quarter == 0 && nblk >= 16 * quarter;
	int bi = blockIdx.x, bstep = nwg, bend = nblk, pair_base = 0;
	if (uneven) {
		const int p = (int)blockIdx.x % quarter, rank = (int)blockIdx.x / quarter;
		const int K2 = 2 * (nblk / quarter);
		const int E = (K2 * a.even_share + 64) >> 7;
		const int g0 = (p & 1) ? E : 0, len = (p & 1) ? K2 - E : E;
		int lo = 0, hi = 0, acc = 0;
#pragma unroll
		for (int r = 0; r < 4; r++) {
			const int nxt = acc + a.share[r];
			if (r == rank) { lo = (len * acc + 32) >> 6; hi = (r == 3) ? len : (len * nxt + 32) >> 6; }
			acc = nxt;
		}
		pair_base = p & ~1;
		bstep = 1;
		bi = g0 + lo;
		bend = g0 + hi;
	}
	auto blk = [&](int i) {
		const int ordinal = uneven ? pair_base + (i & 1) + quarter * (i >> 1) : i;
		return a.forward ? ordinal : nblk - 1 - ordinal;
	};
	if (bi < bend) load_block(v, a_in, a.lda, a.n, blk(bi));
	if constexpr (DEEP) { if (bi + bstep < bend) load_block(v2, a_in, a.lda, a.n, blk(bi + bstep)); }
	if (a.skip_status && a.skip_status[0] != 0) return;
	if constexpr (sizeof(IO) == 2) {
		if (blockIdx.x == 0 && a.r16) {
			_Float16* r16 = reinterpret_cast<_Float16*>(a.r16);
			for (int e = threadIdx.x; e < a.n * a.n; e += 64 * NW) r16[(size_t)(e / a.n) * a.ldr16 + (e % a.n)] = (_Float16)a.r32[e];
		}
	}

	if constexpr (ENGINE == 0) {
		float* Zs = reinterpret_cast<float*>(zbase);
		constexpr int ZE0 = (NP * NP) / (64 * NW);
		static_assert((NP * NP) % (64 * NW) == 0, "Z elements divide evenly over the workgroup");
		float zv0[ZE0];
#pragma unroll
		for (int u = 0; u < ZE0; u++) zv0[u] = a.z[threadIdx.x + u * 64 * NW];
#pragma unroll
		for (int u = 0; u < ZE0; u++) {
			const int idx = threadIdx.x + u * 64 * NW;
			const int k = idx % NP, j = idx / NP;
			if constexpr (ZTRI) {
				const int g = k >> 4;
				if (j >= 16 * g) Zs[ztri_base(g) + (k & 15) * ztri_stride(g) + (j - 16 * g)] = zv0[u];
			} else {
				Zs[k * ZS + j] = zv0[u];
			}
		}
	} else if constexpr (ENGINE == 2) {
		_Float16* Zh = reinterpret_cast<_Float16*>(zbase);
		constexpr int ZE2 = (NB * 64 * 8) / (64 * NW);
		static_assert((NB * 64 * 8) % (64 * NW) == 0, "Z image elements divide evenly over the workgroup");
		float zv2[ZE2];
#pragma unroll
		for (int u = 0; u < ZE2; u++) {
			const int idx = threadIdx.x + u * 64 * NW;
			const int jj = idx & 7, l = (idx >> 3) & 63, b = idx >> 9;
			const int kt = zblk_kt(b), ct = COMPACT ? b - (kt * NT - kt * (kt - 1)) + 2 * kt : b % NT;
			const int k = 32 * kt + 8 * (l >> 4) + jj, j = 16 * ct + (l & 15);
			zv2[u] = a.z[(size_t)j * NP + min(k, NP - 1)];
			if (k >= NP) zv2[u] = 0.0f;
		}
#pragma unroll
		for (int u = 0; u < ZE2; u++) Zh[threadIdx.x + u * 64 * NW] = (_Float16)zv2[u];
	} else {
		unsigned short* Zb = reinterpret_cast<unsigned short*>(zbase);
		constexpr int ZE = (NB * 64 * 8) / (64 * NW);
		static_assert((NB * 64 * 8) % (64 * NW) == 0, "Z image elements divide evenly over the workgroup");
		float zv[ZE];
#pragma unroll
		for (int u = 0; u < ZE; u++) {
			const int idx = threadIdx.x + u * 64 * NW;
			const int jj = idx & 7, l = (idx >> 3) & 63, b = idx >> 9;
			const int kt = zblk_kt(b), ct = COMPACT ? b - (kt * NT - kt * (kt - 1)) + 2 * kt : b % NT;
			const int k = 32 * kt + 8 * (l >> 4) + jj, j = 16 * ct + (l & 15);
			zv[u] = a.z[(size_t)j * NP + min(k, NP - 1)];
			if (k >= NP) zv[u] = 0.0f;
		}
#pragma unroll
		for (int u = 0; u < ZE; u++) {
			const int idx = threadIdx.x + u * 64 * NW;
			unsigned h, m, lo;
			split3(zv[u], h, m, lo);
			Zb[0 * NB * 512 + idx] = (unsigned short)h;
			Zb[1 * NB * 512 + idx] = (unsigned short)m;
			Zb[2 * NB * 512 + idx] = (unsigned short)lo;
		}
	}

	for (; bi < bend; bi += bstep) {
		const int b = blk(bi);
#pragma unroll
		for (int k = 0; k < NI; k++) {
			const int col = (wv + NW * k) * CPI + lcol;
			*reinterpret_cast<f32x4*>(&As[col * RS + (lrow ^ swz(col))]) = v[k];
		}
		__syncthreads();
		if constexpr (DEEP) {
#pragma unroll
			for (int k = 0; k < NI; k++) v[k] = v2[k];
			if (bi + 2 * bstep < bend) load_block(v2, a_in, a.lda, a.n, blk(bi + 2 * bstep));
		} else {
			if (bi + bstep < bend) load_block(v, a_in, a.lda, a.n, blk(bi + bstep));
		}
		f32x4 cin[UPD ? NI : 1];
// ... 406 lines not shown
```

### tsqr_gpu_amd/csrc/tsqr_mi.hip

```cpp
#include <hip/hip_runtime.h>
#include <algorithm>
#include <atomic>
#include <cmath>
#include <cstdio>
#include <cstdlib>
#include <cstring>
#include <dlfcn.h>
#include <string>
#include <vector>

#include "../../include/tsqr_mi.h"
#include "stream_order.h"
#include "tsqr_kernels.hip"
#include "tsqr_wide.hip"
#include "tsqr_f64.hip"
#include "tsqr_f64_wide.hip"
#include "f64_plan.h"
#include "validate.hip"

namespace {

int env_int(const char* name, int dflt) { const char* e = getenv(name); return e ? atoi(e) : dflt; }

struct Settings {
// ... 131 lines not shown

struct WqLayout { size_t z, s, r1, r2, r3, r4, r5, r6, gsum, status, wide, smulti, gmulti, total; };
WqLayout wq_layout(size_t m, size_t n) {
	const Plan p = make_plan(m, n);
	WqLayout L{};
	size_t o = p.stack_b;
	o = (o + 63) & ~(size_t)63;
	L.z = o; o += 4096;
	L.s = o; o += 4096;
	L.r1 = o; o += n * n;
	L.r2 = o; o += n * n;
	L.r3 = o; o += 4096;
	L.r4 = o; o += 4096;
	L.r5 = o; o += 4096;
	L.r6 = o; o += 4096;
	o = (o + 63) & ~(size_t)63;
	L.gsum = o; o += 2 * GSUM_DOUBLES;
	L.status = o; o += 64;
	L.wide = o;
	if (n > PW) o += WIDE_FLOATS;
	o = (o + 63) & ~(size_t)63;
	L.smulti = o; L.gmulti = o;
	if (n > PW) {
		const size_t ntr = cdiv(n, PW) - 1;
		o += ntr * 4096;
		L.gmulti = o; o += ntr * 2 * (size_t)tsqrmi::CROSS_GSTRIDE;
	}
	L.total = o;
	return L;
}

typedef int (*nccl_allgather_t)(const void*, void*, size_t, int, void*, hipStream_t);
typedef int (*nccl_allreduce_t)(const void*, void*, size_t, int, int, void*, hipStream_t);
struct Comm {
	int nranks = 1;
	void* nccl = nullptr;
	nccl_allreduce_t nccl_allreduce = nullptr;
	nccl_allgather_t nccl_allgather = nullptr;
	tsqr_mi_allreduce_f64_cb cb_allreduce = nullptr;
	tsqr_mi_allgather_f32_cb cb_allgather = nullptr;
	void* cb_user = nullptr;
	float* gather_buf = nullptr;
	bool active() const { return nccl != nullptr || cb_allreduce != nullptr; }
	int allreduce_f64(double* buf, size_t count, hipStream_t st) const {
		if (nccl_allreduce) return nccl_allreduce(buf, buf, count, 8 , 0 , nccl, st) == 0 ? 0 : -1;
		if (cb_allreduce) return cb_allreduce(cb_user, buf, count, st) == 0 ? 0 : -1;
		return 0;
	}
	int allgather_f32(const float* send, float* recv, size_t count, hipStream_t st) const {
		if (nccl_allgather) return nccl_allgather(send, recv, count, 7 , nccl, st) == 0 ? 0 : -1;
		if (cb_allgather) return cb_allgather(cb_user, send, recv, count, st) == 0 ? 0 : -1;
		return -1;
	}
};
void* rccl_symbol(const char* name) { return dlsym(RTLD_DEFAULT, name); }

struct HostSig { unsigned* host = nullptr; unsigned* dev = nullptr; };
struct Ctx {
	hipStream_t st = nullptr;
	int dev = 0;
	float* wq = nullptr; float* wr = nullptr;
	WqLayout L{};
	size_t cross_slots = 0;
	HostSig hsig;
	int policy = 0, gram_level = 2;
	int min_level = 2;
	bool used_shift = false, used_householder = false;
	bool wide = true;
	int slot = 0, prev_slot = -1;
	double* gramq_part = nullptr;
	int gramq_cap = 0, gramq_nparts = 0;
	bool gramq_ready = false;
	Comm comm;
	bool fold_cor = false;
	bool resume_accepted = false;
	float resume_scond = 0.0f;
	int start_level = -1;
	unsigned* announce_word = nullptr;
	unsigned announce_seq = 0;
	bool q_for_next_sweep = false;
	int chol_relax = 0;
	int chol_retry_shift = 0;
	double rows_global = 0.0;
	unsigned* status_dev(int s) const { return reinterpret_cast<unsigned*>(wq + L.status) + 16 * s; }
	double* gsum() const { return reinterpret_cast<double*>(wq + L.gsum); }
};
template <class GramArgsT> void carry_announcement(Ctx& c, GramArgsT& ga) {
	ga.announce = c.announce_word; ga.announce_seq = c.announce_seq; c.announce_word = nullptr;
}
void raise_announcement(Ctx& c) {
	if (!c.announce_word) return;
	hipLaunchKernelGGL(tsqrmi::host_flag_kernel, dim3(1), dim3(1), 0, c.st, c.announce_word, c.announce_seq);
	c.announce_word = nullptr;
}

struct OwnPinned {
	unsigned* host = nullptr; unsigned* dev = nullptr;
	~OwnPinned() { if (host) (void)hipHostFree(host); }
	bool get() {
		if (host) return dev != nullptr;
		if (hipHostMalloc(reinterpret_cast<void**>(&host), 64, hipHostMallocDefault) != hipSuccess) { host = nullptr; (void)hipGetLastError(); return false; }
		if (hipHostGetDevicePointer(reinterpret_cast<void**>(&dev), host, 0) != hipSuccess) { dev = nullptr; (void)hipGetLastError(); return false; }
		return true;
	}
};
thread_local OwnPinned t_own;

struct HostSigCache { unsigned* h_wl = nullptr; unsigned* dev = nullptr; };
thread_local HostSigCache t_hsig_cache;
void resolve_host_sig(Ctx& c, unsigned* h_wl, size_t m) {
	c.hsig = HostSig{};
	if (h_wl && ref_bs(m) + 1 >= 8) {
		if (t_hsig_cache.h_wl == h_wl) { c.hsig.host = h_wl; c.hsig.dev = t_hsig_cache.dev; return; }
		hipPointerAttribute_t at{};
		if (hipPointerGetAttributes(&at, h_wl) == hipSuccess && at.type == hipMemoryTypeHost && at.devicePointer) {
			c.hsig.host = h_wl; c.hsig.dev = reinterpret_cast<unsigned*>(at.devicePointer);
			t_hsig_cache.h_wl = h_wl; t_hsig_cache.dev = c.hsig.dev;
			return;
		}
		(void)hipGetLastError();
	}
	if (t_own.get()) { c.hsig.host = t_own.host; c.hsig.dev = t_own.dev; }
}

int wait_word(volatile unsigned* word, unsigned seq, hipStream_t st) {
	for (;;) {
		for (int k = 0; k < 20000; k++) {
			if (*word == seq) return 0;
			__builtin_ia32_pause();
		}
		const hipError_t e = hipStreamQuery(st);
		if (e == hipSuccess) return 0;
		if (e != hipErrorNotReady) HIPCHK(e);
	}
}

int signal_and_wait(Ctx& c) {
	if (!c.hsig.dev || t_prof.on) return 1;
	unsigned seq = ++g_seq;
	if (seq == 0) seq = ++g_seq;
	volatile unsigned* flag = reinterpret_cast<volatile unsigned*>(c.hsig.host) + 3;
	*flag = 0;
	hipLaunchKernelGGL(tsqrmi::host_flag_kernel, dim3(1), dim3(1), 0, c.st, c.hsig.dev + 3, seq);
	if (hipGetLastError() != hipSuccess) return 1;
	return wait_word(flag, seq, c.st);
}
int wait_done(Ctx& c) {
	const int w = signal_and_wait(c);
	if (w < 0) return w;
	if (w == 1) HIPCHK(hipStreamSynchronize(c.st));
	return 0;
}

thread_local tsqr_mi_ticket* t_pending[2] = {nullptr, nullptr};
thread_local unsigned t_submits = 0;
int ticket_latch(tsqr_mi_ticket* t) {
	if (!t || t->pending != 1) return 0;
	volatile unsigned* w = reinterpret_cast<volatile unsigned*>(t->words) + 4 * t->slot;
	const int rc = wait_word(w + 3, t->seq, reinterpret_cast<hipStream_t>(t->stream));
	if (rc) { t_pending[t->slot] = nullptr; t->pending = 0; t->state = -1; return rc; }
	t->verdict = w[0];
	const unsigned b = w[2];
	memcpy(&t->scond, &b, 4);
	t->pending = 2;
	if (t_pending[t->slot] == t) t_pending[t->slot] = nullptr;
	return 0;
}
// ... 38 lines not shown
			else hipLaunchKernelGGL((tsqrmi::fold_kernel<4, true, false>), dim3(blocks), dim3(256), 0, st, a);
			return 0;
		}
	}
	if (a.cor) hipLaunchKernelGGL((tsqrmi::fold_kernel<NT, false, true>), dim3(blocks), dim3(256), 0, st, a);
	else hipLaunchKernelGGL((tsqrmi::fold_kernel<NT, false, false>), dim3(blocks), dim3(256), 0, st, a);
	return 0;
}
int dispatch_fold(int NT, const tsqrmi::FoldArgs& a, hipStream_t st) {
	switch (NT) {
		case 1: return launch_fold<1>(a, st);
		case 2: return launch_fold<2>(a, st);
		case 3: return launch_fold<3>(a, st);
		default: return launch_fold<4>(a, st);
	}
}

int fold_coop(Ctx& c, float* r, size_t ldr, float* stack, size_t stack_ld, int nblocks, size_t n, float* other, bool cor) {
	constexpr int W = tsqrmi::FOLD_COOP_WAVES;
	constexpr int lds = tsqrmi::FOLD_COOP_LDS_FLOATS * (int)sizeof(float);
	static DevOnce attr[2];
	if (attr[cor].need(c.dev)) {
		HIPCHK(hipFuncSetAttribute(cor ? reinterpret_cast<const void*>(&tsqrmi::fold_coop_kernel<true>) : reinterpret_cast<const void*>(&tsqrmi::fold_coop_kernel<false>),
		                           hipFuncAttributeMaxDynamicSharedMemorySize, lds));
		attr[cor].done(c.dev);
	}
	float* cur = stack; size_t cur_ld = stack_ld;
	float* nxt = other;
	for (;;) {
		tsqrmi::FoldTreeArgs a{};
		a.src = cur; a.ld = cur_ld; a.nblocks = nblocks; a.n = (int)n;
		const int wgs = (nblocks + W - 1) / W;
		if (wgs == 1) { a.dst = r; a.dst_ld = ldr; a.rows_store = (int)n; a.cols_store = (int)n; }
		else { a.dst = nxt; a.dst_ld = (size_t)wgs * 64; a.rows_store = 64; a.cols_store = 64; }
		{
			ProfScope ps(KC_TREE, c.st);
			if (cor) hipLaunchKernelGGL(tsqrmi::fold_coop_kernel<true>, dim3(wgs), dim3(64 * W), lds, c.st, a);
			else hipLaunchKernelGGL(tsqrmi::fold_coop_kernel<false>, dim3(wgs), dim3(64 * W), lds, c.st, a);
		}
		HIPCHK(hipGetLastError());
		if (wgs == 1) break;
		float* t = cur; cur = nxt; nxt = t; cur_ld = (size_t)wgs * 64;
		nblocks = wgs;
	}
	return 0;
}

int fold_r(Ctx& c, float* r, size_t ldr, const float* src, size_t ld, size_t m, size_t n, float* stack_a, float* stack_b) {
	const Plan p = make_plan(m, n);
	const int NT = (int)(p.NP / 16);
	const bool cor = c.fold_cor;
	const float* cur = src; size_t cur_ld = ld;
	for (int lv = 0; lv < p.nlevels; lv++) {
		tsqrmi::FoldArgs a{};
		a.src = cur; a.ld = cur_ld; a.m = p.rows[lv];
		a.n = (int)n;
		a.nchunks = p.nch[lv]; a.cpw = p.cpw[lv]; a.nwaves = p.nw[lv];
		a.tri_init = (lv > 0 && p.NP == 64) ? 1 : 0;
		a.cor = cor ? 1 : 0;
		if (p.nw[lv] == 1) {
			a.dst = r; a.dst_ld = ldr; a.rows_store = (int)n; a.cols_store = (int)n;
		} else {
			float* stack = (lv % 2 == 0) ? stack_a : stack_b;
			a.dst = stack; a.dst_ld = (size_t)p.nw[lv] * p.NP; a.rows_store = (int)p.NP; a.cols_store = (int)p.NP;
			cur = stack; cur_ld = a.dst_ld;
		}
		{
			ProfScope ps(lv == 0 ? KC_FOLD0 : KC_TREE, c.st);
			dispatch_fold(NT, a, c.st);
		}
		HIPCHK(hipGetLastError());
		if (lv == 0 && p.nw[0] > 1 && p.NP == 64) {
			return fold_coop(c, r, ldr, stack_a, (size_t)p.nw[0] * 64, p.nw[0], n, stack_b, cor);
		}
	}
	return 0;
}

template <int NT> void launch_gram(const tsqrmi::GramArgs& a, int nblocks, bool bf16, hipStream_t st) {
	if (bf16) hipLaunchKernelGGL(tsqrmi::gram_bf16_kernel<NT>, dim3(nblocks), dim3(256), 0, st, a);
	else hipLaunchKernelGGL(tsqrmi::gram_kernel<NT>, dim3(nblocks), dim3(256), 0, st, a);
}

int gram_g(Ctx& c, const float* src, size_t ld, size_t m, size_t n, bool bf16, bool io_half = false) {
	const GramPlan g = gram_plan(m, n);
	const int NT = (int)(np_of(n) / 16);
	tsqrmi::GramArgs a{};
	a.a = src; a.lda = ld; a.m = m; a.n = (int)n; a.nchunks = g.nch; a.cpw = g.cpw; a.nwaves = g.nwaves;
	a.part = reinterpret_cast<double*>(c.wr);
	a.skip_status = c.prev_slot >= 0 ? c.status_dev(c.prev_slot) : nullptr;
	if (!(bf16 && c.gramq_ready)) carry_announcement(c, a);
	int nparts = g.nblocks;
	if (bf16 && c.gramq_ready) {
		c.gramq_ready = false;
		nparts = c.gramq_nparts;
	} else if (io_half) {
		ProfScope ps(KC_GRAM, c.st);
		switch (NT) {
			case 1: hipLaunchKernelGGL(tsqrmi::gram_h_kernel<1>, dim3(g.nblocks), dim3(256), 0, c.st, a); break;
			case 2: hipLaunchKernelGGL(tsqrmi::gram_h_kernel<2>, dim3(g.nblocks), dim3(256), 0, c.st, a); break;
			case 3: hipLaunchKernelGGL(tsqrmi::gram_h_kernel<3>, dim3(g.nblocks), dim3(256), 0, c.st, a); break;
			default: hipLaunchKernelGGL(tsqrmi::gram_h_kernel<4>, dim3(g.nblocks), dim3(256), 0, c.st, a); break;
		}
	} else if (bf16 && n == 64 && m % 128 == 0 && m <= ((size_t)1 << 20) && ld % 4 == 0 && ld <= ((size_t)1 << 24) && (reinterpret_cast<uintptr_t>(src) & 15) == 0) {
		static DevOnce attr;
		if (attr.need(c.dev)) {
			HIPCHK(hipFuncSetAttribute(reinterpret_cast<const void*>(&tsqrmi::gram_blk_kernel), hipFuncAttributeMaxDynamicSharedMemorySize, tsqrmi::GB_LDS_BYTES));
			attr.done(c.dev);
		}
		a.nchunks = (int)(m / 128);
		nparts = std::min(a.nchunks, g.nblocks);
		ProfScope ps(KC_GRAM, c.st);
		hipLaunchKernelGGL(tsqrmi::gram_blk_kernel, dim3(nparts), dim3(256), tsqrmi::GB_LDS_BYTES, c.st, a);
	} else {
		ProfScope ps(KC_GRAM, c.st);
		switch (NT) {
			case 1: launch_gram<1>(a, g.nblocks, bf16, c.st); break;
			case 2: launch_gram<2>(a, g.nblocks, bf16, c.st); break;
			case 3: launch_gram<3>(a, g.nblocks, bf16, c.st); break;
			default: launch_gram<4>(a, g.nblocks, bf16, c.st); break;
		}
	}
	HIPCHK(hipGetLastError());
	const int nelem = g.ntri * 256;
	{
		ProfScope ps(KC_CHOL, c.st);
		hipLaunchKernelGGL(tsqrmi::gram_reduce1_kernel, dim3((nelem + 15) / 16), dim3(256), 0, c.st, c.gsum(), a.part, nparts, nelem, (double)m,
		                   nullptr, (size_t)0, nullptr, 0);
	}
	HIPCHK(hipGetLastError());
	if (c.comm.active()) {
		ProfScope ps(KC_MISC, c.st);
		if (c.comm.allreduce_f64(c.gsum(), (size_t)nelem + 1, c.st)) { t_last_error = "all-reduce of the Gram tiles failed"; return -1; }
	}
	return 0;
}

int chol_from_g(Ctx& c, float* r, size_t ldr, size_t n, int level) {
	tsqrmi::CholArgs a{};
	a.r = r; a.ldr = ldr; a.z = c.wq + c.L.z;
	a.status = c.status_dev(c.slot);
	a.host_status = c.hsig.dev ? c.hsig.dev + 4 * c.slot : nullptr;
	a.gsum = c.gsum();
	a.prev_status = c.prev_slot >= 0 ? c.status_dev(c.prev_slot) : nullptr;
	const int NT = (int)(np_of(n) / 16);
	a.rows_dev = c.comm.active() ? c.gsum() + (size_t)(NT * (NT + 1) / 2) * 256 : nullptr;
	a.rows = c.rows_global;
	a.shift_coef = (level == 3) ? 11.0 * 1.1102230246251565e-16 : 0.0;
	a.n = (int)n; a.NT = NT; a.level = level; a.scond_floor = g_set.bf16_scond_floor;
	if (level == 2) { a.relax = c.chol_relax; a.retry_shift = c.chol_retry_shift; }
	{
		ProfScope ps(KC_CHOL, c.st);
		hipLaunchKernelGGL(tsqrmi::chol16_kernel, dim3(1), dim3(1024), 0, c.st, a);
	}
	HIPCHK(hipGetLastError());
	return 0;
}

template <int E, int NT, bool UPD, int ROWS, bool GRAMQ> constexpr auto apply_wg_entry() {
	if constexpr (GRAMQ) return &tsqrmi::apply_wg_gramq_kernel<E, NT, UPD, ROWS>;
	else return &tsqrmi::apply_wg_kernel<E, NT, UPD, ROWS>;
}
template <int E, int NT, bool UPD, int ROWS, bool GRAMQ = false> int launch_apply_wg(Ctx& c, tsqrmi::ApplyArgs a) {
	constexpr auto kernel = apply_wg_entry<E, NT, UPD, ROWS, GRAMQ>();
	constexpr int NP = 16 * NT, KT = (NP + 31) / 32;
	constexpr int NB = (!UPD && NT == 4) ? 6 : KT * NT;
	size_t lds = sizeof(float) * NP * (ROWS + 4) +
	             (E == 0 ? sizeof(float) * NP * (NP + 16) : (size_t)(E == 2 ? 1 : 3) * NB * 512 * 2);
	if (GRAMQ) lds = std::max(lds, sizeof(double) * 2 * (NT * (NT + 1) / 2) * 256);
	static DevOnce attr;
	static std::atomic<int> per_cu_cache[MAX_DEV];
	if (attr.need(c.dev)) {
		HIPCHK(hipFuncSetAttribute(reinterpret_cast<const void*>(kernel), hipFuncAttributeMaxDynamicSharedMemorySize, (int)lds));
		int nb = 0;
		if (hipOccupancyMaxActiveBlocksPerMultiprocessor(&nb, reinterpret_cast<const void*>(kernel), 256, lds) != hipSuccess || nb < 1) {
			(void)hipGetLastError(); nb = 2;
		}
		per_cu_cache[c.dev].store(std::min(nb, ROWS == 64 ? 4 : (E == 0 ? 2 : 3)));
		attr.done(c.dev);
	}
	const size_t nblk = cdiv(a.m, (size_t)ROWS);
	a.nchunks = (int)nblk;
	const int wgs = g_set.apply_wgs.load();
	size_t want = wgs > 0 ? (size_t)wgs : (size_t)256 * per_cu_cache[c.dev].load();
	unsigned gy = 1;
	if constexpr (UPD) {
		if (a.multi_cols > 0) { gy = (unsigned)cdiv((size_t)a.multi_cols, PW); want = std::max<size_t>(1, want / gy); }
	}
	a.nwaves = (int)std::min<size_t>(nblk, want);
	a.cpw = 0;
	if constexpr (GRAMQ) {
		a.nwaves = std::min(a.nwaves, c.gramq_cap);
		a.gpart = c.gramq_part;
		c.gramq_nparts = a.nwaves;
	}
	if constexpr (!UPD && !GRAMQ && ROWS == 64) {
		if (a.nwaves == 1024 && per_cu_cache[c.dev].load() == 4) {
			static const int pinned = env_int("TSQR_MI_APPLY_SHARES", -1);
			static std::atomic<int> chosen[MAX_DEV][2];
			auto set_mode = [](tsqrmi::ApplyArgs& x, int mode) {
				x.share[0] = x.share[1] = x.share[2] = x.share[3] = 0; x.even_share = 0;
				if (mode == 1 || mode == 2) { x.share[0] = 18; x.share[1] = 17; x.share[2] = 15; x.share[3] = 14; x.even_share = (mode == 1) ? 69 : 64; }
			};
			const double bytes = (double)a.m * (double)a.n * sizeof(float);
			const int cls = bytes > 256.0 * 1048576.0 ? 1 : 0;
			int mode = pinned == 0 ? 3 : (pinned == 1 ? 1 : (pinned == 2 ? 2 : chosen[c.dev][cls].load()));
			const bool big = bytes >= 128.0 * 1048576.0;
			if (mode == 0 && big && reinterpret_cast<const void*>(a.q) != reinterpret_cast<const void*>(a.a) && !t_prof.on) {
				constexpr int REPS = 4;
				hipEvent_t ev[2 * REPS + 1];
				bool ok = true;
				for (auto& e : ev) ok = ok && hipEventCreate(&e) == hipSuccess;
				if (ok) {
					for (int i = 0; i < 2 * REPS; i++) {
						tsqrmi::ApplyArgs x = a;
						set_mode(x, (i & 1) ? 3 : 1);
						(void)hipEventRecord(ev[i], c.st);
						hipLaunchKernelGGL(kernel, dim3(a.nwaves, gy), dim3(256), lds, c.st, x);
					}
					(void)hipEventRecord(ev[2 * REPS], c.st);
					ok = hipEventSynchronize(ev[2 * REPS]) == hipSuccess;
					float t[2] = {0.f, 0.f};
					for (int i = 0; i < 2 * REPS && ok; i++) { float ms = 0.f; ok = hipEventElapsedTime(&ms, ev[i], ev[i + 1]) == hipSuccess; t[i & 1] += ms; }
					if (ok && t[0] > 0.01f * REPS && t[1] > 0.01f * REPS)
						chosen[c.dev][cls].store(t[0] < 0.99f * t[1] ? 1 : 3);
				}
				for (auto& e : ev) (void)hipEventDestroy(e);
				(void)hipGetLastError();
				return 0;
			}
			set_mode(a, mode == 0 ? 3 : mode);
		}
	}
	hipLaunchKernelGGL(kernel, dim3(a.nwaves, gy), dim3(256), lds, c.st, a);
	return 0;
}
template <int E, int NT, bool UPD> int launch_apply_any(Ctx& c, const tsqrmi::ApplyArgs& a) {
	if constexpr (!UPD && E != 0) {
		if (c.gramq_part && c.gramq_cap > 0) return launch_apply_wg<E, NT, UPD, 128, true>(c, a);
	}
	if constexpr (!UPD && E == 1) return launch_apply_wg<E, NT, UPD, 64>(c, a);
	else return launch_apply_wg<E, NT, UPD, 128>(c, a);
}
template <int E, int NT> int launch_apply_h(Ctx& c, tsqrmi::ApplyArgs a) {
	constexpr int ROWS = (E == 1) ? 64 : 128;
	constexpr auto kernel = &tsqrmi::apply_wg_h_kernel<E, NT, ROWS>;
	constexpr int NP = 16 * NT, KT = (NP + 31) / 32;
	constexpr int NB = (NT == 4) ? 6 : KT * NT;
	const size_t lds = sizeof(float) * NP * (ROWS + 4) + (E == 0 ? sizeof(float) * NP * (NP + 16) : (size_t)(E == 2 ? 1 : 3) * NB * 512 * 2);
	static DevOnce attr;
	static std::atomic<int> per_cu_cache[MAX_DEV];
	if (attr.need(c.dev)) {
		HIPCHK(hipFuncSetAttribute(reinterpret_cast<const void*>(kernel), hipFuncAttributeMaxDynamicSharedMemorySize, (int)lds));
		int nb = 0;
		if (hipOccupancyMaxActiveBlocksPerMultiprocessor(&nb, reinterpret_cast<const void*>(kernel), 256, lds) != hipSuccess || nb < 1) {
			(void)hipGetLastError(); nb = 2;
		}
		per_cu_cache[c.dev].store(std::min(nb, ROWS == 64 ? 4 : 3));
		attr.done(c.dev);
	}
	const size_t nblk = cdiv(a.m, (size_t)ROWS);
	a.nchunks = (int)nblk;
	a.nwaves = (int)std::min<size_t>(nblk, (size_t)256 * per_cu_cache[c.dev].load());
	a.cpw = 0;
	hipLaunchKernelGGL(kernel, dim3(a.nwaves), dim3(256), lds, c.st, a);
	return 0;
}
template <int E> int dispatch_apply_h(Ctx& c, int NT, const tsqrmi::ApplyArgs& a) {
	switch (NT) {
		case 1: return launch_apply_h<E, 1>(c, a);
		case 2: return launch_apply_h<E, 2>(c, a);
		case 3: return launch_apply_h<E, 3>(c, a);
		default: return launch_apply_h<E, 4>(c, a);
	}
}
template <int E> int dispatch_apply_nt(Ctx& c, int NT, const tsqrmi::ApplyArgs& a) {
	switch (NT) {
// ... 795 lines not shown
	explicit Completion(Ctx& ctx) : c(ctx), words(reinterpret_cast<volatile unsigned*>(ctx.hsig.host)) {}
	int close(int i, bool last) {
		unsigned sq = ++g_seq;
		if (sq == 0) sq = ++g_seq;
		seq[i & 1] = sq;
		words[4 * (i & 1) + 3] = 0;
		c.announce_word = c.hsig.dev + 4 * (i & 1) + 3; c.announce_seq = sq;
		if (last) raise_announcement(c);
		HIPCHK(hipGetLastError());
		return 0;
	}
	int wait(int i) const { return wait_word(words + 4 * (i & 1) + 3, seq[i & 1], c.st); }
	bool rejected(int i) const { return words[4 * (i & 1)] != 0; }
};

extern "C++" template <class Step, class Tail>
static int run_chained(const Completion& comp, const Mats& mt, int count, int engine, Step step, Tail tail, int* done) {
	int rc = step(0);
	if (rc) return rc;
	for (int i = 0; i < count; i++) {
		if (i + 1 < count) { rc = step(i + 1); if (rc) return rc; }
		rc = comp.wait(i);
		if (rc) return rc;
		if (comp.rejected(i)) return tail(i);
		mt.state(i, TSQR_MI_SUCCESS);
		*done = i + 1;
	}
	t_last_engine = engine;
	prof_collect();
	return TSQR_MI_SUCCESS;
}

static int blocking_one(const CallEnv& env, const Mats& mt, int i, const Call& cl) {
	if (!env.dist)
		return tsqr_mi_qr_f32(cl.mode, cl.reorth, mt.q(i), cl.ldq, mt.r(i), cl.ldr, mt.a(i), cl.lda, cl.m, cl.n, cl.wq, cl.wr, nullptr, nullptr, cl.h_wl, cl.stream);
	Ctx cc;
	cc.comm = env.comm;
	return qr_dist_common(cc, cl.mode, cl.reorth, mt.q(i), cl.ldq, mt.r(i), cl.ldr, mt.a(i), cl.lda, cl.m, cl.n, cl.wq, cl.wr, env.nranks, cl.stream);
}

static int rejected_tail(const CallEnv& env, const Mats& mt, int count, const Call& cl, int i, const Completion& comp, int* done) {
	HIPCHK(hipStreamSynchronize(comp.c.st));
	prof_collect();
	const bool next = i + 1 < count, next_rejected = next && comp.rejected(i + 1);
	int first = 0;
	if (mt.same()) {
		for (int k = i; k < count; k++) {
			const int s = blocking_one(env, mt, k, cl);
			if (s < 0) return s;
			mt.state(k, s);
			if (s && !first) first = s;
		}
		*done = count;
		return first;
	}
	int s = blocking_one(env, mt, i, cl);
	if (s < 0) return s;
	mt.state(i, s);
	first = s;
	*done = i + 1;
	if (next) {
		s = 0;
		if (next_rejected) { s = blocking_one(env, mt, i + 1, cl); if (s < 0) return s; }
		mt.state(i + 1, s);
		if (s && !first) first = s;
		*done = i + 2;
	}
	return first;
}

static bool blk_shape(const Call& cl) {
	return !cl.reorth && cl.n == PW && cl.m % 128 == 0 && cl.m <= ((size_t)1 << 20) && cl.lda % 4 == 0 && cl.lda <= ((size_t)1 << 24) &&
	       cl.lda >= cl.m && cl.ldq >= cl.m && cl.ldr >= cl.n;
}
static int blk_kernel_attrs(int dev) {
	static DevOnce attr;
	if (attr.need(dev)) {
		HIPCHK(hipFuncSetAttribute(reinterpret_cast<const void*>(&tsqrmi::gram_blk_kernel), hipFuncAttributeMaxDynamicSharedMemorySize, tsqrmi::GB_LDS_BYTES));
		HIPCHK(hipFuncSetAttribute(reinterpret_cast<const void*>(&tsqrmi::gram_blk_chain_kernel), hipFuncAttributeMaxDynamicSharedMemorySize, tsqrmi::GB_LDS_BYTES));
		attr.done(dev);
	}
	return 0;
}
static tsqrmi::GramArgs gram_args_64(Ctx& c, const float* a, const Call& cl, int nchunks, const GramPlan& g, double* part) {
	tsqrmi::GramArgs ga{};
	ga.a = a; ga.lda = cl.lda; ga.m = cl.m; ga.n = (int)cl.n; ga.nchunks = nchunks; ga.cpw = g.cpw; ga.nwaves = g.nwaves;
	ga.part = part;
	carry_announcement(c, ga);
	return ga;
}
static tsqrmi::CholArgs chol_args_64(const Ctx& c, float* r, size_t ldr, int i, size_t n) {
	tsqrmi::CholArgs ca{};
	ca.r = r; ca.ldr = ldr; ca.z = c.wq + c.L.z;
	ca.status = c.status_dev(i & 1);
	ca.host_status = c.hsig.dev + 4 * (i & 1);
	ca.gsum = c.gsum();
	ca.rows = c.rows_global;
	ca.n = (int)n; ca.NT = 4; ca.level = 2; ca.scond_floor = g_set.bf16_scond_floor;
	return ca;
}

static int chained64(const Mats& mt, int count, const Call& cl, int* done) {
	*done = 0;
	const size_t m = cl.m, n = cl.n;
	const int engine = engine_of(cl.mode);
	if (count < 3 || engine < 0 || !blk_shape(cl) || !a_aligned16(mt, count)) return NOT_MINE;
	if (!out_of_order(mt, count, cl) || !chain_fits_cache(mt, cl)) return NOT_MINE;
	Ctx c;
	env_ctx(c, CallEnv{}, cl.wq, cl.wr, m, n, cl.h_wl, cl.stream, false);
	if (!(c.policy == 0 && c.gram_level == 2 && c.hsig.dev && !g_set.debug)) return NOT_MINE;
	c.fold_cor = (engine == 1);
	int rc = blk_kernel_attrs(c.dev);
	if (rc) return rc;
	const GramPlan g = gram_plan(m, n);
	const int nchunks = (int)(m / 128), nparts = std::min(nchunks, g.nblocks), nelem = 10 * 256, nred = nelem / 16;
	double* part[2] = {reinterpret_cast<double*>(c.wr), reinterpret_cast<double*>(c.wr) + (size_t)g.nblocks * nelem};
	unsigned* ticket = c.status_dev(0) + 8;
	HIPCHK(hipMemsetAsync(ticket, 0, sizeof(unsigned), c.st));
	Completion comp(c);
	auto step = [&](int i) -> int {
		if (i + 1 < count) {
			tsqrmi::ChainArgs ch{};
			ch.chol = chol_args_64(c, mt.r(i), cl.ldr, i, n);
			ch.part = part[i & 1]; ch.nparts = nparts; ch.ticket = ticket; ch.nred = nred;
			ProfScope ps(KC_GRAM, c.st);
			hipLaunchKernelGGL(tsqrmi::gram_blk_chain_kernel, dim3(nred + nparts), dim3(256), tsqrmi::GB_LDS_BYTES, c.st,
			                   gram_args_64(c, mt.a(i + 1), cl, nchunks, g, part[(i + 1) & 1]), ch);
		} else {
			raise_announcement(c);
			ProfScope ps(KC_CHOL, c.st);
			hipLaunchKernelGGL(tsqrmi::gram_reduce1_kernel, dim3(nred), dim3(256), 0, c.st, c.gsum(), part[i & 1], nparts, nelem, (double)m,
			                   nullptr, (size_t)0, nullptr, 0);
			hipLaunchKernelGGL(tsqrmi::chol16_kernel, dim3(1), dim3(1024), 0, c.st, chol_args_64(c, mt.r(i), cl.ldr, i, n));
		}
		HIPCHK(hipGetLastError());
		c.slot = i & 1;
		const int rc2 = apply_rinv(c, engine, mt.q(i), cl.ldq, mt.a(i), cl.lda, mt.r(i), cl.ldr, m, n, true, c.status_dev(i & 1));
		return rc2 ? rc2 : comp.close(i, i + 1 == count);
	};
	{
		ProfScope ps(KC_GRAM, c.st);
		hipLaunchKernelGGL(tsqrmi::gram_blk_kernel, dim3(nparts), dim3(256), tsqrmi::GB_LDS_BYTES, c.st, gram_args_64(c, mt.a(0), cl, nchunks, g, part[0]));
	}
	HIPCHK(hipGetLastError());
	return run_chained(comp, mt, count, 3, step, [&](int i) { return rejected_tail(CallEnv{}, mt, count, cl, i, comp, done); }, done);
}

static int chained128(const Mats& mt, int count, const Call& cl, int* done) {
	*done = 0;
	const size_t m = cl.m, n = cl.n, lda = cl.lda, ldq = cl.ldq, ldr = cl.ldr;
	const int engine = engine_of(cl.mode);
	if (count < 3 || engine < 0 || cl.reorth || n != 2 * PW || m < n || m % 64 != 0 || m / 64 < 2 * (size_t)WIDE_MAX_WGS || lda > ((size_t)1 << 23) ||
	    lda < m || ldq < m || ldr < n || lda % 4 != 0 || !a_aligned16(mt, count))
		return NOT_MINE;
	if (!out_of_order(mt, count, cl) || !chain_fits_cache(mt, cl)) return NOT_MINE;
	Ctx c;
	env_ctx(c, CallEnv{}, cl.wq, cl.wr, m, n, cl.h_wl, cl.stream, false);
	if (!(c.wide && c.policy == 0 && c.gram_level == 2 && c.hsig.dev && !g_set.debug)) return NOT_MINE;
	static DevOnce attr;
	if (attr.need(c.dev)) {
		HIPCHK(hipFuncSetAttribute(reinterpret_cast<const void*>(&tsqrmi::gram_wide_kernel<true>), hipFuncAttributeMaxDynamicSharedMemorySize, tsqrmi::GW_LDS_BYTES));
		HIPCHK(hipFuncSetAttribute(reinterpret_cast<const void*>(&tsqrmi::gram_wide_chain_kernel), hipFuncAttributeMaxDynamicSharedMemorySize, tsqrmi::GWC_LDS_BYTES));
		attr.done(c.dev);
	}
	float* w = c.wq + c.L.wide;
	double* gsum = reinterpret_cast<double*>(w);
	float* zw = w + WIDE_OFF_ZW;
	float* zf2 = w + WIDE_OFF_ZF2;
	const int nblk = (int)(m / 64), wgs = WIDE_MAX_WGS, nelem = 36 * 256;
	double* part = reinterpret_cast<double*>(c.wr);
	Completion comp(c);
	auto gram_args = [&](int i) {
		tsqrmi::GramWideArgs ga{};
		ga.a = mt.a(i); ga.lda = lda; ga.m = m; ga.n = (int)n; ga.blk0 = 0; ga.nblk = nblk; ga.part = part;
		carry_announcement(c, ga);
		return ga;
	};
	auto chol_args = [&](int i) {
		tsqrmi::CholWideArgs wa{};
		wa.gsum = gsum; wa.r = mt.r(i); wa.ldr = ldr; wa.n = (int)n; wa.zf1 = c.wq + c.L.z; wa.zf2 = zf2; wa.zw = zw;
		wa.st1 = c.status_dev(2); wa.st2 = c.status_dev(3); wa.status = c.status_dev(i & 1);
		wa.host_status = c.hsig.dev + 4 * (i & 1);
		wa.rows = (double)m; wa.scond_floor = g_set.bf16_scond_floor;
		return wa;
	};
	auto reduce = [&]() {
		ProfScope ps(KC_CHOL, c.st);
		hipLaunchKernelGGL(tsqrmi::gram_reduce1_kernel, dim3(nelem / 16), dim3(256), 0, c.st, gsum, part, wgs, nelem, (double)m, nullptr, (size_t)0, nullptr, 0);
	};
	auto step = [&](int i) -> int {
		if (i + 1 < count) {
			{
				ProfScope ps(KC_GRAM, c.st);
				hipLaunchKernelGGL(tsqrmi::gram_wide_chain_kernel, dim3(1 + wgs), dim3(512), tsqrmi::GWC_LDS_BYTES, c.st, gram_args(i + 1), chol_args(i));
			}
			reduce();
		} else {
			raise_announcement(c);
			ProfScope ps(KC_CHOL, c.st);
			hipLaunchKernelGGL(tsqrmi::chol_wide_kernel, dim3(1), dim3(1024), 0, c.st, chol_args(i));
		}
		HIPCHK(hipGetLastError());
		tsqrmi::ApplyArgs aa{};
		aa.a = mt.a(i); aa.lda = lda; aa.q = mt.q(i); aa.ldq = ldq; aa.m = m; aa.n = (int)n; aa.z = zw; aa.skip_status = c.status_dev(i & 1);
		int rc;
		{
			ProfScope ps(KC_APPLY, c.st);
			rc = (engine == 0) ? launch_apply_wide<0>(c, aa) : (engine == 1 ? launch_apply_wide<1>(c, aa) : launch_apply_wide<2>(c, aa));
		}
		if (rc) return rc;
		HIPCHK(hipGetLastError());
		return comp.close(i, i + 1 == count);
	};
	{
		ProfScope ps(KC_GRAM, c.st);
		hipLaunchKernelGGL((tsqrmi::gram_wide_kernel<true>), dim3(wgs), dim3(512), tsqrmi::GW_LDS_BYTES, c.st, gram_args(0));
	}
	reduce();
	HIPCHK(hipGetLastError());
	return run_chained(comp, mt, count, 5, step, [&](int i) { return rejected_tail(CallEnv{}, mt, count, cl, i, comp, done); }, done);
}

static int chained_dist(const CallEnv& env, const Mats& mt, int count, const Call& cl, int* done) {
	*done = 0;
	const size_t m = cl.m, n = cl.n;
	const int engine = engine_of(cl.mode);
	if (engine < 0 || m == 0 || n == 0 || n > PW || env.nranks < 1 || env.nranks > 255) return NOT_MINE;
	Ctx c;
	env_ctx(c, env, cl.wq, cl.wr, m, n, nullptr, cl.stream, false);
	const bool mine = c.hsig.dev && blk_shape(cl) && c.policy == 0 && c.gram_level == 2 && !g_set.debug && out_of_order(mt, count, cl) && a_aligned16(mt, count);
	c.fold_cor = (engine == 1);
	int rc = blk_kernel_attrs(c.dev);
	if (rc) return rc;
	const GramPlan g = gram_plan(m, PW);
	const int nchunks = (int)(m / 128), nparts = std::min(nchunks, g.nblocks), nelem = 10 * 256;
	double* part = reinterpret_cast<double*>(c.wr);
	Completion comp(c);
	auto chol_args = [&](int i) {
		tsqrmi::CholArgs ca = chol_args_64(c, mt.r(i), cl.ldr, i, n);
		ca.rows_dev = c.gsum() + nelem;
		return ca;
	};
	auto reduce_allreduce = [&](int extra) -> int {
		{
			ProfScope ps(KC_CHOL, c.st);
			hipLaunchKernelGGL(tsqrmi::gram_reduce1_kernel, dim3(nelem / 16), dim3(256), 0, c.st, c.gsum(), part, nparts, nelem, (double)m,
			                   nullptr, (size_t)0, nullptr, 0);
		}
		HIPCHK(hipGetLastError());
		if (extra) hipLaunchKernelGGL(tsqrmi::set_f64_kernel, dim3(1), dim3(1), 0, c.st, c.gsum() + nelem + 1, 1.0);
		ProfScope ps(KC_MISC, c.st);
		if (c.comm.allreduce_f64(c.gsum(), (size_t)nelem + 1 + extra, c.st)) { t_last_error = "all-reduce of the Gram tiles failed"; return -1; }
		return 0;
	};
	if (mine) {
		{
			ProfScope ps(KC_GRAM, c.st);
			hipLaunchKernelGGL(tsqrmi::gram_blk_kernel, dim3(nparts), dim3(256), tsqrmi::GB_LDS_BYTES, c.st, gram_args_64(c, mt.a(0), cl, nchunks, g, part));
		}
		HIPCHK(hipGetLastError());
		rc = reduce_allreduce(1);
	} else {
		HIPCHK(hipMemsetAsync(c.gsum(), 0, sizeof(double) * ((size_t)nelem + 2), c.st));
		if (c.comm.allreduce_f64(c.gsum(), (size_t)nelem + 2, c.st)) { t_last_error = "all-reduce of the schedule flags failed"; rc = -1; }
	}
	if (rc) return rc;
	if (c.hsig.dev) {
		unsigned vs = ++g_seq;
		if ((vs & 0xffffffu) == 0) vs = ++g_seq;
		comp.words[8] = 0;
		hipLaunchKernelGGL(tsqrmi::vote_out_kernel, dim3(1), dim3(1), 0, c.st, c.gsum() + nelem + 1, c.hsig.dev + 8, vs);
		HIPCHK(hipGetLastError());
		unsigned w = 0;
		for (;;) {
			bool seen = false;
			for (int k = 0; k < 20000 && !seen; k++) {
				w = comp.words[8];
				seen = (w >> 8) == (vs & 0xffffffu);
				if (!seen) __builtin_ia32_pause();
			}
			if (seen) break;
			const hipError_t e = hipStreamQuery(c.st);
			if (e == hipSuccess) { w = comp.words[8]; break; }
			if (e != hipErrorNotReady) HIPCHK(e);
		}
		if ((int)(w & 0xffu) != env.nranks || (w >> 8) != (vs & 0xffffffu)) { prof_collect(); return NOT_MINE; }
	} else {
		HIPCHK(hipStreamSynchronize(c.st));
		return NOT_MINE;
	}
	auto step = [&](int i) -> int {
		if (i + 1 < count) {
			tsqrmi::ChainArgs ch{};
			ch.chol = chol_args(i); ch.direct = 1;
			{
				ProfScope ps(KC_GRAM, c.st);
				hipLaunchKernelGGL(tsqrmi::gram_blk_chain_kernel, dim3(1 + nparts), dim3(256), tsqrmi::GB_LDS_BYTES, c.st,
				                   gram_args_64(c, mt.a(i + 1), cl, nchunks, g, part), ch);
			}
			HIPCHK(hipGetLastError());
			const int rc2 = reduce_allreduce(0);
			if (rc2) return rc2;
		} else {
			raise_announcement(c);
			ProfScope ps(KC_CHOL, c.st);
			hipLaunchKernelGGL(tsqrmi::chol16_kernel, dim3(1), dim3(1024), 0, c.st, chol_args(i));
			HIPCHK(hipGetLastError());
		}
		c.slot = i & 1;
		const int rc2 = apply_rinv(c, engine, mt.q(i), cl.ldq, mt.a(i), cl.lda, mt.r(i), cl.ldr, m, n, true, c.status_dev(i & 1));
		return rc2 ? rc2 : comp.close(i, i + 1 == count);
	};
	return run_chained(comp, mt, count, 3, step, [&](int i) { return rejected_tail(env, mt, count, cl, i, comp, done); }, done);
}

static bool attempt_stands(const tsqr_mi_ticket* t) { return t->verdict == 0 && !(t->n <= 16 && t->scond > 32.0f); }
static int two_in_flight(const CallEnv& env, const Mats& mt, int count, const Call& cl) {
	auto submit = [&](int i, tsqr_mi_ticket* t, tsqr_mi_ticket* announce, bool own_flag) {
		return submit_impl(env, cl.mode, cl.reorth, mt.q(i), cl.ldq, mt.r(i), cl.ldr, mt.a(i), cl.lda, cl.m, cl.n, cl.wq, cl.wr, cl.h_wl, cl.stream, t, announce, own_flag);
	};
	const bool redo_after_ladder = mt.same() && (env.dist || [&] { const tsqr_order::Operands o = ops_of(mt, 0, cl, sizeof(float)); return tsqr_order::feeds(o, o); }());
	tsqr_mi_ticket tk[2];
	int first = 0;
	bool ordered = pair_conflicts(mt, count, 0, cl);
	int st = submit(0, &tk[0], nullptr, count == 1 || ordered);
	if (st) { for (int k = 0; k < count; k++) mt.state(k, st); return st; }
	for (int i = 0; i < count; i++) {
		tsqr_mi_ticket* cur = &tk[i & 1];
		tsqr_mi_ticket* nxt = (i + 1 < count) ? &tk[(i + 1) & 1] : nullptr;
		const bool ordered_next = nxt && pair_conflicts(mt, count, i + 1, cl);
		if (nxt && !ordered) {
			st = submit(i + 1, nxt, cur, i + 2 == count || ordered_next);
			if (st) { (void)finish_impl(env, cur); return st; }
		}
		const bool had_attempt = cur->pending != 0;
		st = finish_impl(env, cur);
		mt.state(i, st);
		if (st && !first) first = st;
		if (st < 0 || (st && mt.same())) { if (nxt && !ordered) (void)finish_impl(env, nxt); return st; }
		if (nxt && !ordered && redo_after_ladder && had_attempt && !attempt_stands(cur)) {
			nxt->pending = 0;
			st = nxt->state = blocking_one(env, mt, i + 1, cl);
			if (st < 0) return st;
		}
		if (nxt && ordered) {
			st = submit(i + 1, nxt, nullptr, i + 2 == count || ordered_next);
			if (st) return st;
		}
		ordered = ordered_next;
	}
	return first;
}

static int conflict_on_any_rank(const CallEnv& env, const Mats& mt, int count, const Call& cl, bool* any) {
	bool mine = false;
	for (int i = 0; i + 1 < count && !mine; i++) mine = pair_conflicts(mt, count, i, cl);
	Ctx c;
	env_ctx(c, env, cl.wq, cl.wr, cl.m, cl.n, nullptr, cl.stream, false);
	hipLaunchKernelGGL(tsqrmi::set_f64_kernel, dim3(1), dim3(1), 0, c.st, c.gsum(), mine ? 1.0 : 0.0);
	HIPCHK(hipGetLastError());
	if (c.comm.allreduce_f64(c.gsum(), 1, c.st)) { t_last_error = "all-reduce of the operand-order flag failed"; return -1; }
	double h = 0.0;
	HIPCHK(hipMemcpyAsync(&h, c.gsum(), sizeof(double), hipMemcpyDeviceToHost, c.st));
	HIPCHK(hipStreamSynchronize(c.st));
	*any = h != 0.0;
	return 0;
}

static int stream_of_calls(const CallEnv& env, const Mats& mt, int count, const Call& cl) {
	const int depth = g_set.loop_depth.load();
	int first = 0;
	bool in_order = count < 2 || depth < 2;
	if (!in_order && env.dist && !mt.same()) {
		const int rc = conflict_on_any_rank(env, mt, count, cl, &in_order);
		if (rc) return rc;
	}
	if (in_order) {
		for (int i = 0; i < count; i++) {
			const int st = blocking_one(env, mt, i, cl);
			mt.state(i, st);
			if (st && !first) first = st;
// ... 72 lines not shown
	if (n <= PW && !reorth && g_set.policy.load() == 0 && g_set.gram_level.load() == 2 && aligned16(a, lda) && aligned16(q, ldq)) {
		Ctx c;
		init_ctx(c, wq_v, wr_v, m, n, stream);
		c.rows_global = (double)m;
		resolve_host_sig(c, h_wl, m);
		c.slot = 0; c.prev_slot = -1;
		int rc = gram_g(c, reinterpret_cast<const float*>(a), lda, m, n, true, true);
		if (!rc) rc = chol_from_g(c, r32, n, n, 2);
		if (!rc) rc = apply_rinv(c, engine_of(f16_engine_mode(mode)), reinterpret_cast<float*>(q), ldq, reinterpret_cast<const float*>(a), lda,
		                         r32, n, m, n, true, c.status_dev(0), true, r, ldr);
		if (rc) return rc;
		unsigned status = 1u;
		float scond = 0.0f;
		rc = read_status(c, 0, &status, &scond);
		if (rc) return rc;
		if (status == 0 && !(n <= 16 && scond > 32.0f)) {
			t_last_engine = 3;
			return TSQR_MI_SUCCESS;
		}
	}
	hipLaunchKernelGGL(tsqrmi::widen_f16_kernel, dim3(grid), dim3(256), 0, st, a32, ld32, reinterpret_cast<const _Float16*>(a), lda, m, (int)n,
	                   aligned16(a, lda) ? 1 : 0);
	HIPCHK(hipGetLastError());
	const int rc = tsqr_mi_qr_f32(emode, reorth, q32, ld32, r32, n, a32, ld32, m, n, wq_v, wr_v, nullptr, d_wl, h_wl, stream);
	if (rc) return rc;
	hipLaunchKernelGGL(tsqrmi::narrow_f16_kernel, dim3(grid), dim3(256), 0, st, reinterpret_cast<_Float16*>(q), ldq, q32, ld32, m, (int)n,
	                   aligned16(q, ldq) ? 1 : 0);
	hipLaunchKernelGGL(tsqrmi::narrow_f16_kernel, dim3((unsigned)cdiv(cdiv(n, 8) * n, 256)), dim3(256), 0, st, reinterpret_cast<_Float16*>(r), ldr, r32, n,
	                   n, (int)n, aligned16(r, ldr) ? 1 : 0);
	HIPCHK(hipGetLastError());
	return tsqr_mi_stream_wait(stream);
}

static int stream_of_calls_f16(const Mats& mt, int count, int mode, size_t ldq, size_t ldr, size_t lda,
                               size_t m, size_t n, void* wq_v, void* wr_v, unsigned* h_wl, void* stream) {
	auto aligned16 = [](const void* p, size_t ld) { return (reinterpret_cast<uintptr_t>(p) & 15) == 0 && ld % 8 == 0; };
	const int emode = f16_engine_mode(mode);
	if (emode < 0 || n > m || m == 0 || n == 0 || n > PW || n <= 16 || ldq < m || lda < m || ldr < n) return NOT_MINE;
	for (int i = 0; i < (mt.same() ? 1 : count); i++)
		if (!aligned16(mt.a(i), lda) || !aligned16(mt.q(i), ldq)) return NOT_MINE;
	const Call cl{mode, 0, ldq, ldr, lda, m, n, wq_v, wr_v, h_wl, stream};
	for (int i = 0; i + 1 < count; i++)
		if (pair_conflicts(mt, count, i, cl, sizeof(_Float16))) return NOT_MINE;
	Ctx c;
	env_ctx(c, CallEnv{}, wq_v, wr_v, m, n, h_wl, stream, false);
	if (!(c.policy == 0 && c.gram_level == 2 && c.hsig.dev && !t_prof.on && !g_set.debug)) return NOT_MINE;
	float* r32 = reinterpret_cast<float*>(wq_v) + f16_tail_offset(m, n) + 2 * f16_ld(m) * n;
	const int engine = engine_of(emode);
	Completion comp(c);
	auto apply_and_close = [&](int i) -> int {
		const int rc = apply_rinv(c, engine, mt.q(i), ldq, mt.a(i), lda, r32, n, m, n, true, c.status_dev(i & 1), true, mt.r(i), ldr);
		return rc ? rc : comp.close(i, i + 1 == count);
	};
	auto tail = [&](int i) -> int {
		HIPCHK(hipStreamSynchronize(c.st));
		const bool next_ok = i + 1 < count && !comp.rejected(i + 1);
		int first = 0;
		for (int k = i; k < count; k++) {
			int st = 0;
			if (!(k == i + 1 && next_ok))
				st = tsqr_mi_qr_f16(mode, 0, mt.q(k), ldq, mt.r(k), ldr, mt.a(k), lda, m, n, wq_v, wr_v, nullptr, nullptr, h_wl, stream);
			if (st < 0) return st;
			mt.state(k, st);
			if (st && !first) first = st;
			if (st && mt.same()) return st;
		}
		return first;
	};
	int done = 0;
	if (!(n == PW && count >= 3 && g_set.loop_depth.load() >= 3 && out_of_order(mt, count, cl, sizeof(_Float16)) && chain_fits_cache(mt, cl, sizeof(_Float16)))) {
		auto step = [&](int i) -> int {
			c.slot = i & 1; c.prev_slot = -1;
			int rc = gram_g(c, mt.a(i), lda, m, n, true, true);
			if (!rc) rc = chol_from_g(c, r32, n, n, 2);
			return rc ? rc : apply_and_close(i);
		};
		return run_chained(comp, mt, count, 3, step, tail, &done);
	}
	const GramPlan g = gram_plan(m, n);
	const int nelem = 10 * 256, nred = nelem / 16;
	double* part[2] = {reinterpret_cast<double*>(c.wr), reinterpret_cast<double*>(c.wr) + (size_t)g.nblocks * nelem};
	unsigned* ticket = c.status_dev(0) + 8;
	HIPCHK(hipMemsetAsync(ticket, 0, sizeof(unsigned), c.st));
	hipLaunchKernelGGL(tsqrmi::gram_h_kernel<4>, dim3(g.nblocks), dim3(256), 0, c.st, gram_args_64(c, mt.a(0), cl, g.nch, g, part[0]));
	HIPCHK(hipGetLastError());
	auto step = [&](int i) -> int {
		c.slot = i & 1; c.prev_slot = -1;
		if (i + 1 < count) {
			tsqrmi::ChainArgs ch{};
			ch.chol = chol_args_64(c, r32, n, i, n);
			ch.part = part[i & 1]; ch.nparts = g.nblocks; ch.ticket = ticket; ch.nred = nred;
			hipLaunchKernelGGL(tsqrmi::gram_h_chain_kernel, dim3(nred + g.nblocks), dim3(256), 0, c.st, gram_args_64(c, mt.a(i + 1), cl, g.nch, g, part[(i + 1) & 1]), ch);
		} else {
			raise_announcement(c);
			hipLaunchKernelGGL(tsqrmi::gram_reduce1_kernel, dim3(nred), dim3(256), 0, c.st, c.gsum(), part[i & 1], g.nblocks, nelem, (double)m,
			                   nullptr, (size_t)0, nullptr, 0);
			hipLaunchKernelGGL(tsqrmi::chol16_kernel, dim3(1), dim3(1024), 0, c.st, chol_args_64(c, r32, n, i, n));
		}
		HIPCHK(hipGetLastError());
		return apply_and_close(i);
	};
	return run_chained(comp, mt, count, 3, step, tail, &done);
}

static int calls_f16(const Mats& mt, int count, int mode, int reorth, size_t ldq, size_t ldr, size_t lda, size_t m, size_t n,
                     void* wq_v, void* wr_v, void* reorth_w, unsigned* d_wl, unsigned* h_wl, void* stream) {
	if (count >= 2 && g_set.loop_depth.load() >= 2 && !reorth) {
		const int st = stream_of_calls_f16(mt, count, mode, ldq, ldr, lda, m, n, wq_v, wr_v, h_wl, stream);
		if (st != NOT_MINE) return st;
	}
	int first = 0;
	for (int i = 0; i < count; i++) {
		const int st = tsqr_mi_qr_f16(mode, reorth, mt.q(i), ldq, mt.r(i), ldr, mt.a(i), lda, m, n, wq_v, wr_v, reorth_w, d_wl, h_wl, stream);
		mt.state(i, st);
		if (st && !first) first = st;
		if (st < 0 || (st && mt.same())) return st;
	}
	return first;
}
int tsqr_mi_qr_f16_loop(int count, int mode, int reorth, void* q, size_t ldq, void* r, size_t ldr, const void* a, size_t lda,
                        size_t m, size_t n, void* wq_v, void* wr_v, void* reorth_w, unsigned* d_wl, unsigned* h_wl, void* stream) {
	const Mats mt = one_triple(reinterpret_cast<float*>(q), reinterpret_cast<float*>(r), const_cast<float*>(reinterpret_cast<const float*>(a)));
	return calls_f16(mt, count, mode, reorth, ldq, ldr, lda, m, n, wq_v, wr_v, reorth_w, d_wl, h_wl, stream);
}
int tsqr_mi_qr_f16_batch(int count, int mode, int reorth, void* const* q, size_t ldq, void* const* r, size_t ldr, const void* const* a, size_t lda,
                         size_t m, size_t n, void* wq_v, void* wr_v, void* reorth_w, unsigned* d_wl, unsigned* h_wl, void* stream, int* states) {
	Mats mt;
	if (const int rc = triple_per_call(mt, count, reinterpret_cast<float* const*>(q), reinterpret_cast<float* const*>(r),
	                                   reinterpret_cast<float* const*>(const_cast<void* const*>(a)), states)) return rc;
	return calls_f16(mt, count, mode, reorth, ldq, ldr, lda, m, n, wq_v, wr_v, reorth_w, d_wl, h_wl, stream);
}

static int env_of_nccl(CallEnv& env, void* nccl_comm, void* nccl_allreduce_fn, void* nccl_allgather_fn, float* gather_buf, int nranks) {
	if (!nccl_comm || !nccl_allreduce_fn || !nccl_allgather_fn) {
		t_last_error = "row-partitioned call needs an ncclComm_t and the ncclAllReduce / ncclAllGather entry points of the library that created it";
		return TSQR_MI_ERROR_UNSUPPORTED;
	}
	env.dist = true; env.nranks = nranks;
	env.comm.nccl = nccl_comm;
	env.comm.nccl_allreduce = reinterpret_cast<nccl_allreduce_t>(nccl_allreduce_fn);
	env.comm.nccl_allgather = reinterpret_cast<nccl_allgather_t>(nccl_allgather_fn);
	env.comm.gather_buf = gather_buf;
	return 0;
}
static int env_of_callbacks(CallEnv& env, tsqr_mi_allreduce_f64_cb allreduce, tsqr_mi_allgather_f32_cb allgather, void* user, float* gather_buf, int nranks) {
	if (!allreduce || !allgather) return TSQR_MI_ERROR_UNSUPPORTED;
	env.dist = true; env.nranks = nranks;
	env.comm.cb_allreduce = allreduce; env.comm.cb_allgather = allgather; env.comm.cb_user = user;
	env.comm.gather_buf = gather_buf;
	return 0;
}
int tsqr_mi_qr_f32_dist_fn(int mode, int reorth, float* q, size_t ldq, float* r, size_t ldr, float* a, size_t lda,
                           size_t m_local, size_t n, void* wq_v, void* wr_v, float* gather_buf,
                           void* nccl_comm, void* nccl_allreduce_fn, void* nccl_allgather_fn, int nranks, void* stream) {
	CallEnv env;
	if (const int rc = env_of_nccl(env, nccl_comm, nccl_allreduce_fn, nccl_allgather_fn, gather_buf, nranks)) return rc;
	return blocking_one(env, one_triple(q, r, a), 0, Call{mode, reorth, ldq, ldr, lda, m_local, n, wq_v, wr_v, nullptr, stream});
}
int tsqr_mi_qr_f32_dist(int mode, int reorth, float* q, size_t ldq, float* r, size_t ldr, float* a, size_t lda,
                        size_t m_local, size_t n, void* wq_v, void* wr_v, float* gather_buf,
                        void* nccl_comm, int nranks, void* stream) {
	void* ar = rccl_symbol("ncclAllReduce");
	void* ag = rccl_symbol("ncclAllGather");
	if (!ar || !ag) {
		t_last_error = "ncclAllReduce / ncclAllGather are not in the global symbol scope (the caller does not link RCCL): "
		               "pass the entry points of the library that created the communicator to tsqr_mi_qr_f32_dist_fn";
		return TSQR_MI_ERROR_UNSUPPORTED;
	}
	return tsqr_mi_qr_f32_dist_fn(mode, reorth, q, ldq, r, ldr, a, lda, m_local, n, wq_v, wr_v, gather_buf, nccl_comm, ar, ag, nranks, stream);
}
int tsqr_mi_qr_f32_dist_cb(int mode, int reorth, float* q, size_t ldq, float* r, size_t ldr, float* a, size_t lda,
                           size_t m_local, size_t n, void* wq_v, void* wr_v, float* gather_buf,
                           tsqr_mi_allreduce_f64_cb allreduce, tsqr_mi_allgather_f32_cb allgather, void* user, int nranks, void* stream) {
	CallEnv env;
	if (const int rc = env_of_callbacks(env, allreduce, allgather, user, gather_buf, nranks)) return rc;
	return blocking_one(env, one_triple(q, r, a), 0, Call{mode, reorth, ldq, ldr, lda, m_local, n, wq_v, wr_v, nullptr, stream});
}
int tsqr_mi_qr_f32_dist_fn_loop(int count, int mode, int reorth, float* q, size_t ldq, float* r, size_t ldr, float* a, size_t lda,
                                size_t m_local, size_t n, void* wq_v, void* wr_v, float* gather_buf,
                                void* nccl_comm, void* nccl_allreduce_fn, void* nccl_allgather_fn, int nranks, void* stream) {
	CallEnv env;
	if (const int rc = env_of_nccl(env, nccl_comm, nccl_allreduce_fn, nccl_allgather_fn, gather_buf, nranks)) return rc;
	return stream_of_calls(env, one_triple(q, r, a), count, Call{mode, reorth, ldq, ldr, lda, m_local, n, wq_v, wr_v, nullptr, stream});
}
int tsqr_mi_qr_f32_dist_cb_loop(int count, int mode, int reorth, float* q, size_t ldq, float* r, size_t ldr, float* a, size_t lda,
                                size_t m_local, size_t n, void* wq_v, void* wr_v, float* gather_buf,
                                tsqr_mi_allreduce_f64_cb allreduce, tsqr_mi_allgather_f32_cb allgather, void* user, int nranks, void* stream) {
	CallEnv env;
	if (const int rc = env_of_callbacks(env, allreduce, allgather, user, gather_buf, nranks)) return rc;
	return stream_of_calls(env, one_triple(q, r, a), count, Call{mode, reorth, ldq, ldr, lda, m_local, n, wq_v, wr_v, nullptr, stream});
}

int tsqr_mi_qr_f32_dist_fn_batch(int count, int mode, int reorth, float* const* q, size_t ldq, float* const* r, size_t ldr, float* const* a, size_t lda,
                                 size_t m_local, size_t n, void* wq_v, void* wr_v, float* gather_buf,
                                 void* nccl_comm, void* nccl_allreduce_fn, void* nccl_allgather_fn, int nranks, void* stream, int* states) {
	CallEnv env;
	if (const int rc = env_of_nccl(env, nccl_comm, nccl_allreduce_fn, nccl_allgather_fn, gather_buf, nranks)) return rc;
	Mats mt;
	if (const int rc = triple_per_call(mt, count, q, r, a, states)) return rc;
	return stream_of_calls(env, mt, count, Call{mode, reorth, ldq, ldr, lda, m_local, n, wq_v, wr_v, nullptr, stream});
}
int tsqr_mi_qr_f32_dist_cb_batch(int count, int mode, int reorth, float* const* q, size_t ldq, float* const* r, size_t ldr, float* const* a, size_t lda,
                                 size_t m_local, size_t n, void* wq_v, void* wr_v, float* gather_buf,
                                 tsqr_mi_allreduce_f64_cb allreduce, tsqr_mi_allgather_f32_cb allgather, void* user, int nranks, void* stream, int* states) {
	CallEnv env;
	if (const int rc = env_of_callbacks(env, allreduce, allgather, user, gather_buf, nranks)) return rc;
	Mats mt;
	if (const int rc = triple_per_call(mt, count, q, r, a, states)) return rc;
	return stream_of_calls(env, mt, count, Call{mode, reorth, ldq, ldr, lda, m_local, n, wq_v, wr_v, nullptr, stream});
}

int tsqr_mi_local_r_f32(float* r, size_t ldr, const float* a, size_t lda, size_t m, size_t n,
                        void* wq, void* wr, void* stream) {
	if (m == 0 || n == 0 || n > PW) return TSQR_MI_ERROR_INVALID_SIZE;
	Ctx c;
	init_ctx(c, wq, wr, m, n, stream);
	return fold_r(c, r, ldr, a, lda, m, n, c.wr, c.wq);
}

int tsqr_mi_apply_rinv_f32(int mode, float* q, size_t ldq, const float* a, size_t lda, const float* r, size_t ldr,
                           size_t m, size_t n, void* wq, void* stream) {
	if (m == 0 || n == 0 || n > PW) return TSQR_MI_ERROR_INVALID_SIZE;
	const int engine = engine_of(mode);
	if (engine < 0) return TSQR_MI_ERROR_UNSUPPORTED;
	Ctx c;
	init_ctx(c, wq, nullptr, m, n, stream);
	return apply_rinv(c, engine, q, ldq, a, lda, r, ldr, m, n);
}

size_t tsqr_mi_gram_elems(size_t n) { const size_t NT = np_of(n) / 16; return NT * (NT + 1) / 2 * 256; }

int tsqr_mi_gram_f32(int level, double* gsum, const float* a, size_t lda, size_t m, size_t n, void* wq, void* wr, void* stream) {
	if (m == 0 || n == 0 || n > PW || (level != 1 && level != 2)) return TSQR_MI_ERROR_INVALID_SIZE;
	Ctx c;
	init_ctx(c, wq, wr, m, n, stream);
	const int rc = gram_g(c, a, lda, m, n, level == 2);
	if (rc) return rc;
	if (gsum && gsum != c.gsum())
		HIPCHK(hipMemcpyAsync(gsum, c.gsum(), sizeof(double) * tsqr_mi_gram_elems(n), hipMemcpyDeviceToDevice, c.st));
	return 0;
}

int tsqr_mi_chol_f32(int level, float* r, size_t ldr, const double* gsum, size_t m, size_t n, void* wq_v, unsigned* status_out, void* stream) {
	if (m == 0 || n == 0 || n > PW || (level != 1 && level != 2 && level != 3)) return TSQR_MI_ERROR_INVALID_SIZE;
	Ctx c;
	init_ctx(c, wq_v, nullptr, m, n, stream);
	c.rows_global = (double)m;
	if (gsum && gsum != c.gsum())
		HIPCHK(hipMemcpyAsync(c.gsum(), gsum, sizeof(double) * tsqr_mi_gram_elems(n), hipMemcpyDeviceToDevice, c.st));
	int rc = chol_from_g(c, r, ldr, n, level);
	if (rc) return rc;
	if (!status_out) return 0;
	unsigned status = 0;
	rc = read_status(c, 0, &status);
	if (rc) return rc;
	*status_out = status;
	return 0;
}

int tsqr_mi_stream_wait(void* stream) {
	Ctx c;
	c.st = reinterpret_cast<hipStream_t>(stream);
	if (t_own.get()) { c.hsig.host = t_own.host; c.hsig.dev = t_own.dev; }
	return wait_done(c);
}

int tsqr_mi_chol_status(const void* wq_v, size_t m, size_t n, unsigned* status_out, void* stream) {
	if (m == 0 || n == 0 || n > PW || !status_out) return TSQR_MI_ERROR_INVALID_SIZE;
	Ctx c;
	init_ctx(c, const_cast<void*>(wq_v), nullptr, m, n, stream);
	return read_status(c, 0, status_out);
}

int tsqr_mi_apply_z_f32(int mode, float* q, size_t ldq, const float* a, size_t lda, size_t m, size_t n, void* wq_v, void* stream) {
	if (m == 0 || n == 0 || n > PW) return TSQR_MI_ERROR_INVALID_SIZE;
	const int engine = engine_of(mode);
	if (engine < 0) return TSQR_MI_ERROR_UNSUPPORTED;
	Ctx c;
	init_ctx(c, wq_v, nullptr, m, n, stream);
	const unsigned* skip = (c.policy == 0) ? c.status_dev(0) : nullptr;
	return apply_rinv(c, engine, q, ldq, a, lda, nullptr, 0, m, n, true, skip);
}

int tsqr_mi_validate_f32(const float* q, size_t ldq, const float* r, size_t ldr, const float* a, size_t lda,
                         size_t m, size_t n, double* scratch, double* out_host, double* gram_out_host, void* stream) {
	if (m == 0 || n == 0 || n > m) return TSQR_MI_ERROR_INVALID_SIZE;
	hipStream_t st = reinterpret_cast<hipStream_t>(stream);
	double* g = scratch;
	double* sums = scratch + n * n;
	HIPCHK(hipMemsetAsync(scratch, 0, sizeof(double) * (n * n + 8), st));
	const size_t rows_per_block = 32 * std::max<size_t>(1, cdiv(cdiv(m, 32), 2048));
	hipLaunchKernelGGL(tsqrmi::gramd_kernel, dim3((unsigned)cdiv(m, rows_per_block)), dim3(256), 0, st, g, q, ldq, m, (int)n, rows_per_block);
	hipLaunchKernelGGL(tsqrmi::orth_sums_kernel, dim3(1), dim3(256), 0, st, sums, g, (int)n);
	if (r && a) hipLaunchKernelGGL(tsqrmi::resid_kernel, dim3((unsigned)cdiv(m, 256)), dim3(256), 0, st, sums, q, ldq, r, ldr, a, lda, m, (int)n);
	HIPCHK(hipGetLastError());
	HIPCHK(hipMemcpyAsync(out_host, sums, sizeof(double) * 5, hipMemcpyDeviceToHost, st));
	if (gram_out_host) HIPCHK(hipMemcpyAsync(gram_out_host, g, sizeof(double) * n * n, hipMemcpyDeviceToHost, st));
	HIPCHK(hipStreamSynchronize(st));
	return 0;
}

int tsqr_mi_rmul_f32(float* r, size_t ldr, const float* r2, size_t ldr2, size_t n, void* wq, void* stream) {
	if (n == 0) return TSQR_MI_ERROR_INVALID_SIZE;
	hipStream_t st = reinterpret_cast<hipStream_t>(stream);
	float* r1 = reinterpret_cast<float*>(wq);
	const unsigned gb = (unsigned)std::min<size_t>(1024, cdiv(n * n, 256));
	hipLaunchKernelGGL(tsqrmi::copy2d_kernel, dim3(gb), dim3(256), 0, st, r1, n, r, ldr, (int)n, (int)n);
	launch_rmul(r, ldr, r2, ldr2, r1, n, n, st);
	HIPCHK(hipGetLastError());
	return 0;
}

}

namespace {

constexpr int F64_MAX_SWEEPS = 6;

thread_local int t_sweeps64 = 0;
thread_local OwnPinned t_own64;

int f64_factor(hipStream_t st, double* wq, double* wr, const double* src, size_t ld, size_t m, size_t n, double* r, size_t ldr,
               bool first, int slot) {
	const F64Plan g = f64_plan(m, n);
	if (g.nblocks <= 0) { t_last_error = "fp64 Gram pass without partials"; return TSQR_MI_ERROR_INVALID_SIZE; }
	const tsqrmi::GramArgs64 ga{src, ld, m, (int)n, g.nch, g.nwaves, wr};
	f64_gram_launch(st, g, ga);
	HIPCHK(hipGetLastError());
	const int nelem = g.ntri * 256;
	hipLaunchKernelGGL(tsqrmi::gram_reduce1_kernel, dim3((nelem + 15) / 16), dim3(256), 0, st, wq + F64_GSUM, wr, g.nblocks, nelem, (double)m,
	                   nullptr, (size_t)0, nullptr, 0);
	HIPCHK(hipGetLastError());
	tsqrmi::CholArgs64 ca{};
	ca.r = r; ca.ldr = ldr; ca.z = wq + F64_Z;
	ca.status = reinterpret_cast<unsigned*>(wq + F64_STATUS) + 4 * slot;
	ca.host_status = t_own64.dev + 4 * slot;
	ca.gsum = wq + F64_GSUM;
	const F64Rule rule = f64_rule(m, n, first);
	ca.shift_coef = rule.shift_coef; ca.max_scond = rule.max_scond; ca.alone_max = rule.alone_max;
// ... 182 lines not shown
```

Before: 91300 GFLOP/s.

## Fuse Gram partial reduction with Cholesky via last-block ticket kernel

```diff
diff --git a/include/tsqr_mi.h b/include/tsqr_mi.h
--- a/include/tsqr_mi.h
+++ b/include/tsqr_mi.h
@@ -100,6 +100,9 @@
 size_t tsqr_mi_gram_elems(size_t n);
 int tsqr_mi_gram_f32(int level, double* gsum, const float* a, size_t lda, size_t m, size_t n, void* wq, void* wr, void* stream);
 int tsqr_mi_chol_f32(int level, float* r, size_t ldr, const double* gsum, size_t m, size_t n, void* wq, unsigned* status_out, void* stream);
+enum { TSQR_MI_FACTOR_RELAX = 1, TSQR_MI_FACTOR_RETRY_SHIFT = 2, TSQR_MI_FACTOR_SHIFTED = 4, TSQR_MI_FACTOR_SPLIT = 8, TSQR_MI_FACTOR_AFTER_REJECTED = 16 };
+int tsqr_mi_factor_f32(int level, int flags, float* r, size_t ldr, double* gsum, float* z, unsigned* words_out,
+                       const float* a, size_t lda, size_t m, size_t n, void* wq, void* wr, void* stream);
 int tsqr_mi_chol_status(const void* wq, size_t m, size_t n, unsigned* status_out, void* stream);
 int tsqr_mi_stream_wait(void* stream);
 int tsqr_mi_apply_z_f32(int mode, float* q, size_t ldq, const float* a, size_t lda, size_t m, size_t n, void* wq, void* stream);
diff --git a/tsqr_gpu_amd/blockqr.py b/tsqr_gpu_amd/blockqr.py
--- a/tsqr_gpu_amd/blockqr.py
+++ b/tsqr_gpu_amd/blockqr.py
@@ -32,7 +32,7 @@
     "tsqr_mi_qr_f32", "tsqr_mi_local_r_f32", "tsqr_mi_apply_rinv_f32", "tsqr_mi_rmul_f32",
     "tsqr_mi_qr_f32_dist", "tsqr_mi_set_tuning", "tsqr_mi_profile_enable", "tsqr_mi_profile_read",
     "tsqr_mi_set_policy", "tsqr_mi_last_engine", "tsqr_mi_set_tuning2",
-    "tsqr_mi_gram_elems", "tsqr_mi_gram_f32", "tsqr_mi_chol_f32", "tsqr_mi_chol_status", "tsqr_mi_stream_wait", "tsqr_mi_apply_z_f32", "tsqr_mi_validate_f32",
+    "tsqr_mi_gram_elems", "tsqr_mi_gram_f32", "tsqr_mi_factor_f32", "tsqr_mi_chol_f32", "tsqr_mi_chol_status", "tsqr_mi_stream_wait", "tsqr_mi_apply_z_f32", "tsqr_mi_validate_f32",
     "tsqr_mi_working_q_size_dist", "tsqr_mi_working_r_size_dist", "tsqr_mi_qr_f32_dist_cb",
     "tsqr_mi_qr_f32_loop", "tsqr_mi_qr_f32_dist_fn", "tsqr_mi_qr_f32_dist_fn_loop", "tsqr_mi_qr_f32_dist_cb_loop",
     "tsqr_mi_qr_f16", "tsqr_mi_qr_f16_loop", "tsqr_mi_working_q_size_f16", "tsqr_mi_working_r_size_f16",
@@ -99,6 +99,8 @@
     L.tsqr_mi_gram_f32.argtypes = [ci, vp, vp, sz, sz, sz, vp, vp, vp]
     L.tsqr_mi_chol_f32.restype = ci
     L.tsqr_mi_chol_f32.argtypes = [ci, vp, sz, vp, sz, sz, vp, ctypes.POINTER(ctypes.c_uint), vp]
+    L.tsqr_mi_factor_f32.restype = ci
+    L.tsqr_mi_factor_f32.argtypes = [ci, ci, vp, sz, vp, vp, ctypes.POINTER(ctypes.c_uint), vp, sz, sz, sz, vp, vp, vp]
     L.tsqr_mi_chol_status.restype = ci
     L.tsqr_mi_chol_status.argtypes = [vp, sz, sz, ctypes.POINTER(ctypes.c_uint), vp]
     L.tsqr_mi_stream_wait.restype = ci
diff --git a/tsqr_gpu_amd/csrc/tsqr_kernels.hip b/tsqr_gpu_amd/csrc/tsqr_kernels.hip
--- a/tsqr_gpu_amd/csrc/tsqr_kernels.hip
+++ b/tsqr_gpu_amd/csrc/tsqr_kernels.hip
@@ -531,10 +531,15 @@
 	const unsigned* skip_status;
 	unsigned* announce; unsigned announce_seq;
 	int old_share;
+	unsigned* arm_ticket;
 };
 
 __device__ __forceinline__ void announce_previous_call(unsigned* word, unsigned seq) {
 	if (word && blockIdx.x == 0 && threadIdx.x == 0) *reinterpret_cast<volatile unsigned*>(word) = seq;
+}
+
+__device__ __forceinline__ void arm_chain_ticket(unsigned* ticket) {
+	if (ticket && blockIdx.x == 0 && threadIdx.x == 0) *ticket = 0u;
 }
 
 template <int NT>
@@ -542,6 +547,7 @@
 	constexpr int NTRI = (NT * (NT + 1)) / 2;
 	__shared__ double red[2][NTRI * 256];
 	announce_previous_call(a.announce, a.announce_seq);
+	arm_chain_ticket(a.arm_ticket);
 	if (a.skip_status && a.skip_status[0] != 0) return;
 	const int lane = threadIdx.x & 63;
 	const int wv = threadIdx.x >> 6;
@@ -606,6 +612,7 @@
 	constexpr int NTRI = (NT * (NT + 1)) / 2;
 	__shared__ double red[2][NTRI * 256];
 	announce_previous_call(a.announce, a.announce_seq);
+	arm_chain_ticket(a.arm_ticket);
 	if (a.skip_status && a.skip_status[0] != 0) return;
 	const int lane = threadIdx.x & 63;
 	const int wv = threadIdx.x >> 6;
@@ -793,6 +800,7 @@
 	constexpr int NTRI = (NT * (NT + 1)) / 2;
 	__shared__ double red[2][NTRI * 256];
 	announce_previous_call(a.announce, a.announce_seq);
+	arm_chain_ticket(a.arm_ticket);
 	gram_h_body<NT>(a, red, blockIdx.x);
 }
 
@@ -927,15 +935,16 @@
 __global__ __launch_bounds__(256, 2) void gram_blk_kernel(const GramArgs a) {
 	extern __shared__ __attribute__((aligned(16))) float gb_as[];
 	announce_previous_call(a.announce, a.announce_seq);
+	arm_chain_ticket(a.arm_ticket);
 	gram_blk_body(a, gb_as, blockIdx.x, gridDim.x);
 }
 
 template <bool WT = false>
-__device__ __forceinline__ void gram_reduce1_body(const int blk, double (*red)[17], double* __restrict__ gout, const double* __restrict__ part,
-                                                  int nparts, int nelem, double rows, float* __restrict__ fin_r, size_t fin_ldr,
-                                                  float* __restrict__ fin_zneg, int fin_ny) {
-	if (blk == 0 && threadIdx.x == 0) gout[nelem] = rows;
-	const int e = threadIdx.x & 15, s = threadIdx.x >> 4;
+__device__ __forceinline__ void gram_reduce1_body(const int blk, const int tid, double (*red)[17], double* __restrict__ gout,
+                                                  const double* __restrict__ part, int nparts, int nelem, double rows,
+                                                  float* __restrict__ fin_r, size_t fin_ldr, float* __restrict__ fin_zneg, int fin_ny) {
+	if (blk == 0 && tid == 0) gout[nelem] = rows;
+	const int e = tid & 15, s = tid >> 4;
 	const int el = blk * 16 + e;
 	double s0 = 0.0, s1 = 0.0, s2 = 0.0, s3 = 0.0;
 	if (el < nelem) {
@@ -989,7 +998,7 @@
                                                            double rows, float* __restrict__ fin_r = nullptr, size_t fin_ldr = 0,
                                                            float* __restrict__ fin_zneg = nullptr, int fin_ny = 0) {
 	__shared__ double red[16][17];
-	gram_reduce1_body<false>(blockIdx.x, red, gout, part, nparts, nelem, rows, fin_r, fin_ldr, fin_zneg, fin_ny);
+	gram_reduce1_body<false>(blockIdx.x, threadIdx.x, red, gout, part, nparts, nelem, rows, fin_r, fin_ldr, fin_zneg, fin_ny);
 }
 
 __device__ __forceinline__ double bcast_lane_f64(double x, int lane_const) {
@@ -1244,14 +1253,15 @@
 	int retry_shift;
 };
 
-__global__ __launch_bounds__(1024) void chol16_kernel(const CholArgs a) {
-	if (a.prev_status && a.prev_status[0] != 0) {
-		if (threadIdx.x == 0) {
-			a.status[0] = 1u; a.status[1] = 0u; a.status[2] = 0u;
-			if (a.host_status) { volatile unsigned* hs = a.host_status; hs[1] = 0u; hs[2] = 0u; hs[0] = 1u; }
-		}
-		return;
-	}
+__device__ __forceinline__ bool chol16_prev_rejected(const CholArgs& a) { return a.prev_status && a.prev_status[0] != 0; }
+__device__ __forceinline__ void chol16_report_rejected(const CholArgs& a) {
+	if (threadIdx.x == 0) {
+		a.status[0] = 1u; a.status[1] = 0u; a.status[2] = 0u;
+		if (a.host_status) { volatile unsigned* hs = a.host_status; hs[1] = 0u; hs[2] = 0u; hs[0] = 1u; }
+	}
+}
+template <class LOADG>
+__device__ __forceinline__ void chol16_run(const CholArgs& a, LOADG loadg) {
 	const double rows = a.rows_dev ? a.rows_dev[0] : a.rows;
 	float min_ratio = 0.0f, max_scond = INFINITY;
 	double min_diag = 0.0, shift = 0.0;
@@ -1266,7 +1276,6 @@
 		shift = a.shift_coef * (rows * (double)a.n + (double)a.n * (double)(a.n + 1));
 	}
 	const bool retry = a.level == 2 && a.retry_shift != 0;
-	auto loadg = [&](int e) { return a.gsum[e]; };
 	chol_body16(a.r, a.ldr, a.z, a.status, retry ? nullptr : a.host_status, loadg, a.n, a.NT, a.level == 2 ? 1 : 0, min_ratio, max_scond, shift, min_diag);
 	if (!retry) return;
 	__shared__ unsigned again;
@@ -1285,6 +1294,10 @@
 		hs[2] = a.status[2];
 		hs[0] = (a.status[0] == 0u && a.status[3] != 0u) ? 2u : a.status[0];
 	}
+}
+__global__ __launch_bounds__(1024) void chol16_kernel(const CholArgs a) {
+	if (chol16_prev_rejected(a)) { chol16_report_rejected(a); return; }
+	chol16_run(a, [&](int e) { return a.gsum[e]; });
 }
 
 template <int U>
@@ -1446,6 +1459,7 @@
 	extern __shared__ __attribute__((aligned(16))) float gb_as[];
 	static_assert(GB_LDS_BYTES >= (int)sizeof(double) * (64 * 65 + 4 * 256 + 128), "chol_body4's arrays alias the block buffers");
 	announce_previous_call(a.announce, a.announce_seq);
+	arm_chain_ticket(a.arm_ticket);
 	const int nchain = ch.direct ? 1 : ch.nred;
 	if ((int)blockIdx.x >= nchain) {
 		gram_blk_body(a, gb_as, (int)blockIdx.x - nchain, (int)gridDim.x - nchain);
@@ -1460,7 +1474,7 @@
 		           rows * 0x1p-90, reinterpret_cast<double*>(gb_as));
 		return;
 	}
-	gram_reduce1_body<true>(blockIdx.x, reinterpret_cast<double (*)[17]>(gb_as), const_cast<double*>(c.gsum), ch.part, ch.nparts, 10 * 256, c.rows,
+	gram_reduce1_body<true>(blockIdx.x, threadIdx.x, reinterpret_cast<double (*)[17]>(gb_as), const_cast<double*>(c.gsum), ch.part, ch.nparts, 10 * 256, c.rows,
 	                        nullptr, 0, nullptr, 0);
 	asm volatile("s_waitcnt vmcnt(0)" ::: "memory");
 	__syncthreads();
@@ -1480,12 +1494,13 @@
 	__shared__ double hc_lds[64 * 65 + 4 * 256 + 128];
 	static_assert(sizeof(hc_lds) >= sizeof(double) * 2 * 10 * 256, "the Gram role's workgroup sum fits");
 	announce_previous_call(a.announce, a.announce_seq);
+	arm_chain_ticket(a.arm_ticket);
 	if ((int)blockIdx.x >= ch.nred) {
 		gram_h_body<4>(a, reinterpret_cast<double (*)[10 * 256]>(hc_lds), (int)blockIdx.x - ch.nred);
 		return;
 	}
 	const CholArgs& c = ch.chol;
-	gram_reduce1_body<true>(blockIdx.x, reinterpret_cast<double (*)[17]>(hc_lds), const_cast<double*>(c.gsum), ch.part, ch.nparts, 10 * 256, c.rows,
+	gram_reduce1_body<true>(blockIdx.x, threadIdx.x, reinterpret_cast<double (*)[17]>(hc_lds), const_cast<double*>(c.gsum), ch.part, ch.nparts, 10 * 256, c.rows,
 	                        nullptr, 0, nullptr, 0);
 	asm volatile("s_waitcnt vmcnt(0)" ::: "memory");
 	__syncthreads();
@@ -1499,6 +1514,34 @@
 	const double* g = c.gsum;
 	chol_body4(c.r, c.ldr, c.z, c.status, c.host_status, [&](int e) { return __hip_atomic_load(&g[e], __ATOMIC_RELAXED, __HIP_MEMORY_SCOPE_AGENT); }, c.n, c.NT,
 	           1, 0.03125f, max_scond, 0.0, rows * 0x1p-90, hc_lds);
+}
+
+struct Chain16Args {
+	CholArgs chol;
+	const double* part; int nparts;
+	int nelem;
+	double rows_local;
+	unsigned* ticket;
+};
+__global__ __launch_bounds__(1024) void chain16_kernel(const Chain16Args ch) {
+	const CholArgs& c = ch.chol;
+	if (chol16_prev_rejected(c)) {
+		if (blockIdx.x == 0) chol16_report_rejected(c);
+		return;
+	}
+	__shared__ double red[4][16][17];
+	const int quarter = threadIdx.x >> 8;
+	gram_reduce1_body<true>((int)blockIdx.x * 4 + quarter, (int)(threadIdx.x & 255), red[quarter], const_cast<double*>(c.gsum), ch.part, ch.nparts,
+	                        ch.nelem, ch.rows_local, nullptr, 0, nullptr, 0);
+	asm volatile("s_waitcnt vmcnt(0)" ::: "memory");
+	__syncthreads();
+	__shared__ unsigned last;
+	if (threadIdx.x == 0) last = (__hip_atomic_fetch_add(ch.ticket, 1u, __ATOMIC_RELAXED, __HIP_MEMORY_SCOPE_AGENT) == gridDim.x - 1u) ? 1u : 0u;
+	__syncthreads();
+	if (!last) return;
+	if (threadIdx.x == 0) __hip_atomic_store(ch.ticket, 0u, __ATOMIC_RELAXED, __HIP_MEMORY_SCOPE_AGENT);
+	const double* g = c.gsum;
+	chol16_run(c, [&](int e) { return __hip_atomic_load(&g[e], __ATOMIC_RELAXED, __HIP_MEMORY_SCOPE_AGENT); });
 }
 
 struct CrossArgs {
@@ -1594,7 +1637,7 @@
                                                                  float* __restrict__ fin_r, size_t fin_ldr, float* __restrict__ fin_zneg, int ny_total) {
 	__shared__ double red[16][17];
 	const int j = blockIdx.y;
-	gram_reduce1_body<false>(blockIdx.x, red, gout + (size_t)j * CROSS_GSTRIDE, part + (size_t)j * nparts * (16 * 256), nparts, 16 * 256, rows,
+	gram_reduce1_body<false>(blockIdx.x, threadIdx.x, red, gout + (size_t)j * CROSS_GSTRIDE, part + (size_t)j * nparts * (16 * 256), nparts, 16 * 256, rows,
 	                         fin_zneg ? fin_r + (size_t)j * 64 * fin_ldr : nullptr, fin_ldr, fin_zneg ? fin_zneg + (size_t)j * 4096 : nullptr,
 	                         min(64, ny_total - 64 * j));
 }
@@ -1684,6 +1727,7 @@
 	int n_out;
 	int multi_cols;
 	double* gpart;
+	unsigned* arm_ticket;
 	const unsigned* skip_status;
 	const float* r32; void* r16; size_t ldr16;
 	int share[4];
@@ -1781,6 +1825,9 @@
 	};
 	if (bi < bend) load_block(v, a_in, a.lda, a.n, blk(bi));
 	if constexpr (DEEP) { if (bi + bstep < bend) load_block(v2, a_in, a.lda, a.n, blk(bi + bstep)); }
+	if constexpr (GRAMQ) {
+		if (a.arm_ticket && blockIdx.x == 0 && blockIdx.y == 0 && threadIdx.x == 0) { a.arm_ticket[0] = 0u; a.arm_ticket[16] = 0u; }
+	}
 	if (a.skip_status && a.skip_status[0] != 0) return;
 	if constexpr (sizeof(IO) == 2) {
 		if (blockIdx.x == 0 && a.r16) {
diff --git a/tsqr_gpu_amd/csrc/tsqr_mi.hip b/tsqr_gpu_amd/csrc/tsqr_mi.hip
--- a/tsqr_gpu_amd/csrc/tsqr_mi.hip
+++ b/tsqr_gpu_amd/csrc/tsqr_mi.hip
@@ -237,7 +237,10 @@
 	int chol_relax = 0;
 	int chol_retry_shift = 0;
 	double rows_global = 0.0;
+	struct PendingReduce { const double* part = nullptr; int nparts = 0, nelem = 0; double rows = 0.0; bool armed = false; } pend;
+	bool gramq_armed = false;
 	unsigned* status_dev(int s) const { return reinterpret_cast<unsigned*>(wq + L.status) + 16 * s; }
+	unsigned* chain_ticket(int s) const { return status_dev(s) + 12; }
 	double* gsum() const { return reinterpret_cast<double*>(wq + L.gsum); }
 };
 template <class GramArgsT> void carry_announcement(Ctx& c, GramArgsT& ga) {
@@ -442,6 +445,25 @@
 	else hipLaunchKernelGGL(tsqrmi::gram_kernel<NT>, dim3(nblocks), dim3(256), 0, st, a);
 }
 
+int flush_reduction(Ctx& c) {
+	if (!c.pend.part) return 0;
+	const Ctx::PendingReduce p = c.pend;
+	c.pend = Ctx::PendingReduce{};
+	{
+		ProfScope ps(KC_CHOL, c.st);
+		hipLaunchKernelGGL(tsqrmi::gram_reduce1_kernel, dim3((p.nelem + 15) / 16), dim3(256), 0, c.st, c.gsum(), p.part, p.nparts, p.nelem, p.rows,
+		                   nullptr, (size_t)0, nullptr, 0);
+	}
+	HIPCHK(hipGetLastError());
+	return 0;
+}
+void launch_chain16(hipStream_t st, const tsqrmi::CholArgs& ca, const double* part, int nparts, int nelem, double rows_local, unsigned* ticket) {
+	tsqrmi::Chain16Args ch{};
+	ch.chol = ca; ch.part = part; ch.nparts = nparts; ch.nelem = nelem; ch.rows_local = rows_local; ch.ticket = ticket;
+	const int groups = (nelem + 15) / 16;
+	hipLaunchKernelGGL(tsqrmi::chain16_kernel, dim3((groups + 3) / 4), dim3(1024), 0, st, ch);
+}
+
 int gram_g(Ctx& c, const float* src, size_t ld, size_t m, size_t n, bool bf16, bool io_half = false) {
 	const GramPlan g = gram_plan(m, n);
 	const int NT = (int)(np_of(n) / 16);
@@ -450,10 +472,13 @@
 	a.part = reinterpret_cast<double*>(c.wr);
 	a.skip_status = c.prev_slot >= 0 ? c.status_dev(c.prev_slot) : nullptr;
 	if (!(bf16 && c.gramq_ready)) carry_announcement(c, a);
+	a.arm_ticket = c.chain_ticket(c.slot);
+	bool armed = true;
 	int nparts = g.nblocks;
 	if (bf16 && c.gramq_ready) {
 		c.gramq_ready = false;
 		nparts = c.gramq_nparts;
+		armed = c.gramq_armed;
 	} else if (io_half) {
 		ProfScope ps(KC_GRAM, c.st);
 		switch (NT) {
@@ -482,14 +507,11 @@
 		}
 	}
 	HIPCHK(hipGetLastError());
-	const int nelem = g.ntri * 256;
-	{
-		ProfScope ps(KC_CHOL, c.st);
-		hipLaunchKernelGGL(tsqrmi::gram_reduce1_kernel, dim3((nelem + 15) / 16), dim3(256), 0, c.st, c.gsum(), a.part, nparts, nelem, (double)m,
-		                   nullptr, (size_t)0, nullptr, 0);
-	}
-	HIPCHK(hipGetLastError());
+	c.pend.part = a.part; c.pend.nparts = nparts; c.pend.nelem = g.ntri * 256; c.pend.rows = (double)m; c.pend.armed = armed;
 	if (c.comm.active()) {
+		const int nelem = c.pend.nelem;
+		const int rc = flush_reduction(c);
+		if (rc) return rc;
 		ProfScope ps(KC_MISC, c.st);
 		if (c.comm.allreduce_f64(c.gsum(), (size_t)nelem + 1, c.st)) { t_last_error = "all-reduce of the Gram tiles failed"; return -1; }
 	}
@@ -509,7 +531,14 @@
 	a.shift_coef = (level == 3) ? 11.0 * 1.1102230246251565e-16 : 0.0;
 	a.n = (int)n; a.NT = NT; a.level = level; a.scond_floor = g_set.bf16_scond_floor;
 	if (level == 2) { a.relax = c.chol_relax; a.retry_shift = c.chol_retry_shift; }
-	{
+	if (c.pend.part && c.pend.armed && !c.comm.active()) {
+		const Ctx::PendingReduce p = c.pend;
+		c.pend = Ctx::PendingReduce{};
+		ProfScope ps(KC_CHOL, c.st);
+		launch_chain16(c.st, a, p.part, p.nparts, p.nelem, p.rows, c.chain_ticket(c.slot));
+	} else {
+		const int rc = flush_reduction(c);
+		if (rc) return rc;
 		ProfScope ps(KC_CHOL, c.st);
 		hipLaunchKernelGGL(tsqrmi::chol16_kernel, dim3(1), dim3(1024), 0, c.st, a);
 	}
@@ -553,6 +582,8 @@
 		a.nwaves = std::min(a.nwaves, c.gramq_cap);
 		a.gpart = c.gramq_part;
 		c.gramq_nparts = a.nwaves;
+		a.arm_ticket = c.chain_ticket(0);
+		c.gramq_armed = true;
 	}
 	if constexpr (!UPD && !GRAMQ && ROWS == 64) {
 		if (a.nwaves == 1024 && per_cu_cache[c.dev].load() == 4) {
@@ -1514,10 +1545,11 @@
 	}
 	return 0;
 }
-static tsqrmi::GramArgs gram_args_64(Ctx& c, const float* a, const Call& cl, int nchunks, const GramPlan& g, double* part) {
+static tsqrmi::GramArgs gram_args_64(Ctx& c, const float* a, const Call& cl, int nchunks, const GramPlan& g, double* part, int slot) {
 	tsqrmi::GramArgs ga{};
 	ga.a = a; ga.lda = cl.lda; ga.m = cl.m; ga.n = (int)cl.n; ga.nchunks = nchunks; ga.cpw = g.cpw; ga.nwaves = g.nwaves;
 	ga.part = part;
+	ga.arm_ticket = c.chain_ticket(slot);
 	carry_announcement(c, ga);
 	return ga;
 }
@@ -1557,13 +1589,11 @@
 			ch.part = part[i & 1]; ch.nparts = nparts; ch.ticket = ticket; ch.nred = nred;
 			ProfScope ps(KC_GRAM, c.st);
 			hipLaunchKernelGGL(tsqrmi::gram_blk_chain_kernel, dim3(nred + nparts), dim3(256), tsqrmi::GB_LDS_BYTES, c.st,
-			                   gram_args_64(c, mt.a(i + 1), cl, nchunks, g, part[(i + 1) & 1]), ch);
+			                   gram_args_64(c, mt.a(i + 1), cl, nchunks, g, part[(i + 1) & 1], (i + 1) & 1), ch);
 		} else {
 			raise_announcement(c);
 			ProfScope ps(KC_CHOL, c.st);
-			hipLaunchKernelGGL(tsqrmi::gram_reduce1_kernel, dim3(nred), dim3(256), 0, c.st, c.gsum(), part[i & 1], nparts, nelem, (double)m,
-			                   nullptr, (size_t)0, nullptr, 0);
-			hipLaunchKernelGGL(tsqrmi::chol16_kernel, dim3(1), dim3(1024), 0, c.st, chol_args_64(c, mt.r(i), cl.ldr, i, n));
+			launch_chain16(c.st, chol_args_64(c, mt.r(i), cl.ldr, i, n), part[i & 1], nparts, nelem, (double)m, c.chain_ticket(i & 1));
 		}
 		HIPCHK(hipGetLastError());
 		c.slot = i & 1;
@@ -1572,7 +1602,7 @@
 	};
 	{
 		ProfScope ps(KC_GRAM, c.st);
-		hipLaunchKernelGGL(tsqrmi::gram_blk_kernel, dim3(nparts), dim3(256), tsqrmi::GB_LDS_BYTES, c.st, gram_args_64(c, mt.a(0), cl, nchunks, g, part[0]));
+		hipLaunchKernelGGL(tsqrmi::gram_blk_kernel, dim3(nparts), dim3(256), tsqrmi::GB_LDS_BYTES, c.st, gram_args_64(c, mt.a(0), cl, nchunks, g, part[0], 0));
 	}
 	HIPCHK(hipGetLastError());
 	return run_chained(comp, mt, count, 3, step, [&](int i) { return rejected_tail(CallEnv{}, mt, count, cl, i, comp, done); }, done);
@@ -1688,7 +1718,7 @@
 	if (mine) {
 		{
 			ProfScope ps(KC_GRAM, c.st);
-			hipLaunchKernelGGL(tsqrmi::gram_blk_kernel, dim3(nparts), dim3(256), tsqrmi::GB_LDS_BYTES, c.st, gram_args_64(c, mt.a(0), cl, nchunks, g, part));
+			hipLaunchKernelGGL(tsqrmi::gram_blk_kernel, dim3(nparts), dim3(256), tsqrmi::GB_LDS_BYTES, c.st, gram_args_64(c, mt.a(0), cl, nchunks, g, part, 0));
 		}
 		HIPCHK(hipGetLastError());
 		rc = reduce_allreduce(1);
@@ -1728,7 +1758,7 @@
 			{
 				ProfScope ps(KC_GRAM, c.st);
 				hipLaunchKernelGGL(tsqrmi::gram_blk_chain_kernel, dim3(1 + nparts), dim3(256), tsqrmi::GB_LDS_BYTES, c.st,
-				                   gram_args_64(c, mt.a(i + 1), cl, nchunks, g, part), ch);
+				                   gram_args_64(c, mt.a(i + 1), cl, nchunks, g, part, (i + 1) & 1), ch);
 			}
 			HIPCHK(hipGetLastError());
 			const int rc2 = reduce_allreduce(0);
@@ -1967,7 +1997,7 @@
 	double* part[2] = {reinterpret_cast<double*>(c.wr), reinterpret_cast<double*>(c.wr) + (size_t)g.nblocks * nelem};
 	unsigned* ticket = c.status_dev(0) + 8;
 	HIPCHK(hipMemsetAsync(ticket, 0, sizeof(unsigned), c.st));
-	hipLaunchKernelGGL(tsqrmi::gram_h_kernel<4>, dim3(g.nblocks), dim3(256), 0, c.st, gram_args_64(c, mt.a(0), cl, g.nch, g, part[0]));
+	hipLaunchKernelGGL(tsqrmi::gram_h_kernel<4>, dim3(g.nblocks), dim3(256), 0, c.st, gram_args_64(c, mt.a(0), cl, g.nch, g, part[0], 0));
 	HIPCHK(hipGetLastError());
 	auto step = [&](int i) -> int {
 		c.slot = i & 1; c.prev_slot = -1;
@@ -1975,12 +2005,10 @@
 			tsqrmi::ChainArgs ch{};
 			ch.chol = chol_args_64(c, r32, n, i, n);
 			ch.part = part[i & 1]; ch.nparts = g.nblocks; ch.ticket = ticket; ch.nred = nred;
-			hipLaunchKernelGGL(tsqrmi::gram_h_chain_kernel, dim3(nred + g.nblocks), dim3(256), 0, c.st, gram_args_64(c, mt.a(i + 1), cl, g.nch, g, part[(i + 1) & 1]), ch);
+			hipLaunchKernelGGL(tsqrmi::gram_h_chain_kernel, dim3(nred + g.nblocks), dim3(256), 0, c.st, gram_args_64(c, mt.a(i + 1), cl, g.nch, g, part[(i + 1) & 1], (i + 1) & 1), ch);
 		} else {
 			raise_announcement(c);
-			hipLaunchKernelGGL(tsqrmi::gram_reduce1_kernel, dim3(nred), dim3(256), 0, c.st, c.gsum(), part[i & 1], g.nblocks, nelem, (double)m,
-			                   nullptr, (size_t)0, nullptr, 0);
-			hipLaunchKernelGGL(tsqrmi::chol16_kernel, dim3(1), dim3(1024), 0, c.st, chol_args_64(c, r32, n, i, n));
+			launch_chain16(c.st, chol_args_64(c, r32, n, i, n), part[i & 1], g.nblocks, nelem, (double)m, c.chain_ticket(i & 1));
 		}
 		HIPCHK(hipGetLastError());
 		return apply_and_close(i);
@@ -2119,7 +2147,8 @@
 	if (m == 0 || n == 0 || n > PW || (level != 1 && level != 2)) return TSQR_MI_ERROR_INVALID_SIZE;
 	Ctx c;
 	init_ctx(c, wq, wr, m, n, stream);
-	const int rc = gram_g(c, a, lda, m, n, level == 2);
+	int rc = gram_g(c, a, lda, m, n, level == 2);
+	if (!rc) rc = flush_reduction(c);
 	if (rc) return rc;
 	if (gsum && gsum != c.gsum())
 		HIPCHK(hipMemcpyAsync(gsum, c.gsum(), sizeof(double) * tsqr_mi_gram_elems(n), hipMemcpyDeviceToDevice, c.st));
@@ -2140,6 +2169,41 @@
 	rc = read_status(c, 0, &status);
 	if (rc) return rc;
 	*status_out = status;
+	return 0;
+}
+
+int tsqr_mi_factor_f32(int level, int flags, float* r, size_t ldr, double* gsum, float* z, unsigned* words_out,
+                       const float* a, size_t lda, size_t m, size_t n, void* wq, void* wr, void* stream) {
+	if (m == 0 || n == 0 || n > PW || (level != 1 && level != 2) || !words_out) return TSQR_MI_ERROR_INVALID_SIZE;
+	Ctx c;
+	init_ctx(c, wq, wr, m, n, stream);
+	c.rows_global = (double)m;
+	if (t_own.get()) { c.hsig.host = t_own.host; c.hsig.dev = t_own.dev; }
+	if (level == 2) { c.chol_relax = (flags & TSQR_MI_FACTOR_RELAX) ? 1 : 0; c.chol_retry_shift = (flags & TSQR_MI_FACTOR_RETRY_SHIFT) ? 1 : 0; }
+	c.slot = 0;
+	if (flags & TSQR_MI_FACTOR_AFTER_REJECTED) {
+		const unsigned one = 1u;
+		HIPCHK(hipMemcpyAsync(c.status_dev(1), &one, sizeof(one), hipMemcpyHostToDevice, c.st));
+		HIPCHK(hipStreamSynchronize(c.st));
+		c.prev_slot = 1;
+	}
+	int rc = gram_g(c, a, lda, m, n, level == 2);
+	if (rc) return rc;
+	const unsigned nparts = (unsigned)c.pend.nparts;
+	const bool merged = !(flags & TSQR_MI_FACTOR_SPLIT) && c.pend.armed;
+	if (!merged) { rc = flush_reduction(c); if (rc) return rc; }
+	rc = chol_from_g(c, r, ldr, n, (flags & TSQR_MI_FACTOR_SHIFTED) && level == 1 ? 3 : level);
+	if (rc) return rc;
+	rc = wait_done(c);
+	if (rc) return rc;
+	const size_t NP = np_of(n);
+	if (gsum) HIPCHK(hipMemcpy(gsum, c.gsum(), sizeof(double) * (tsqr_mi_gram_elems(n) + 1), hipMemcpyDeviceToDevice));
+	if (z) HIPCHK(hipMemcpy(z, c.wq + c.L.z, sizeof(float) * NP * NP, hipMemcpyDeviceToDevice));
+	HIPCHK(hipMemcpy(words_out, c.status_dev(0), 4 * sizeof(unsigned), hipMemcpyDeviceToHost));
+	for (int k = 0; k < 3; k++) words_out[4 + k] = c.hsig.host ? reinterpret_cast<volatile unsigned*>(c.hsig.host)[k] : 0xffffffffu;
+	HIPCHK(hipMemcpy(words_out + 7, c.chain_ticket(0), sizeof(unsigned), hipMemcpyDeviceToHost));
+	words_out[8] = nparts;
+	words_out[9] = merged ? 1u : 0u;
 	return 0;
 }
 
```

Result: slower. 89850 GFLOP/s (-1.6%).
